# PaddleCV-SIG/MedicalSeg

Hardware: AMD Instinct MI355X
Metric: 3D-voxels/sec fwd+bwd, VNet 128^3 fp32 (higher is better)
Workload: dtype f32

## Files before the change

include/msegk.h:

```cpp
#ifndef MSEGK_H
#define MSEGK_H

#include <stddef.h>
#include <stdint.h>

#ifdef __cplusplus
extern "C" {
#endif

typedef struct msk_ctx msk_ctx;

typedef struct {
  void* p;
  int32_t n, d, h, w, c;
  int32_t ld;
} msk_tensor;

typedef struct {
  int32_t kd, kh, kw;
  int32_t sd, sh, sw;
  int32_t pd, ph, pw;
} msk_conv_desc;

int msk_version(void);
// ... 95 lines not shown
                               msk_tensor dy_scratch, msk_tensor dx, int dx_accumulate, float* dw, int dw_accumulate,
                               const void* xform , void* ybuf , const float* maxes ,
                               msk_tensor dx_lo, msk_tensor dx_hi, int* split_done);
int msk_conv3d_bwd_bnact_acc(msk_ctx* ctx, msk_conv_desc cd, msk_tensor x, const float* w, msk_tensor y, const float* scale,
                             const float* shift, const float* alpha, const float* mean, const float* invstd, const float* gamma,
                             msk_tensor dout, const float* sums_total, double M_total, msk_tensor dy_scratch, msk_tensor dx,
                             int dx_accumulate, float* dw, int dw_accumulate, const void* xform, void* ybuf, const float* maxes,
                             msk_tensor dx_old, msk_tensor dx_lo, msk_tensor dx_hi, int* split_done);
int msk_conv3d_bwd_bnact_join(msk_ctx* ctx, msk_conv_desc cd, msk_tensor x, const float* w, msk_tensor y, const float* scale,
                              const float* shift, const float* alpha , const float* mean, const float* invstd,
                              const float* gamma, msk_tensor dout, const float* sums_total, double M_total, msk_tensor dy,
                              float* dy_amax , float* dw, int dw_accumulate, const void* xform ,
                              const float* x_amax , msk_tensor jy, const float* jscale, const float* jshift,
                              const float* jalpha_inner, msk_tensor jres, const float* jalpha_outer, const float* jmean,
                              const float* jinvstd, msk_tensor da, int da_accumulate, msk_tensor dres ,
                              int dres_accumulate, float* dalpha_outer, float* unit_sums, float* maxes, int clear_maxes,
                              float* unit_dgamma , float* unit_dbeta , float* unit_dalpha );
int msk_convT3d_bwd_bnact(msk_ctx* ctx, msk_conv_desc cd, msk_tensor x, const float* w, msk_tensor y, const float* scale,
                          const float* shift, const float* alpha , const float* mean, const float* invstd,
                          msk_tensor dout, const float* sums_total, double M_total, msk_tensor dy_scratch, msk_tensor dx,
                          int dx_accumulate, float* dw, int dw_accumulate);
int msk_conv3d_bwd_inact(msk_ctx* ctx, msk_conv_desc cd, msk_tensor x, const float* w, msk_tensor y, const float* scale,
                         const float* shift, const float* alpha , const float* mean, const float* invstd, int coef_stride,
                         msk_tensor dout, const float* sums, int sums_stride, double M_sample, msk_tensor dx, int dx_accumulate,
                         float* dw, int dw_accumulate, const void* xform, void* ybuf, const float* maxes );
int msk_conv3d_bwd_bnact_c1(msk_ctx* ctx, msk_conv_desc cd, msk_tensor x, msk_tensor y, const float* scale, const float* shift,
                            const float* alpha , const float* mean, const float* invstd, msk_tensor res,
                            msk_tensor dout, const float* sums_total, double M_total, float* dw, int dw_accumulate);
int msk_conv3d_dgrad(msk_ctx* ctx, msk_conv_desc cd, msk_tensor dy, const float* w,
                     msk_tensor dx, int accumulate);
int msk_conv3d_wgrad(msk_ctx* ctx, msk_conv_desc cd, msk_tensor x, msk_tensor dy,
                     float* dw, float* db , int accumulate);
int msk_convT3d_fwd(msk_ctx* ctx, msk_conv_desc cd, msk_tensor x, const float* w,
                    const float* bias , msk_tensor y);
int msk_convT3d_fwd_ex(msk_ctx* ctx, msk_conv_desc cd, msk_tensor x, const float* w, const float* bias, msk_tensor y,
                       float* stats_local, const msk_bn_fin* fin );
int msk_convT3d_dgrad(msk_ctx* ctx, msk_conv_desc cd, msk_tensor dy, const float* w,
                      msk_tensor dx, int accumulate);
int msk_convT3d_wgrad(msk_ctx* ctx, msk_conv_desc cd, msk_tensor x, msk_tensor dy,
                      float* dw, float* db , int accumulate);

int msk_bn_stats(msk_ctx* ctx, msk_tensor x, float* stats_local);
int msk_bn_finalize(msk_ctx* ctx, const float* gathered, int world, double count_per_rank,
                    int C, const float* gamma, const float* beta, float eps, float momentum,
                    float* running_mean, float* running_var, float* save_mean,
                    float* save_invstd, float* scale, float* shift);
int msk_bn_eval_coeffs(msk_ctx* ctx, int C, const float* gamma, const float* beta,
                       const float* running_mean, const float* running_var, float eps,
                       float* save_mean, float* save_invstd, float* scale, float* shift);
int msk_affine_act_fwd(msk_ctx* ctx, msk_tensor x, const float* scale, const float* shift,
                       msk_tensor res, const float* alpha, msk_tensor out);
int msk_affine_act_fwd_amax2(msk_ctx* ctx, msk_tensor x, const float* scale, const float* shift, msk_tensor res,
                             const float* alpha, msk_tensor out, float* out_amax , msk_tensor out2);
int msk_affine_act_bwd_reduce(msk_ctx* ctx, msk_tensor x, const float* scale, const float* shift,
                              msk_tensor res, const float* alpha, const float* mean,
                              const float* invstd, msk_tensor dout, float* sums);
int msk_affine_act_bwd_reduce_ex(msk_ctx* ctx, msk_tensor x, const float* scale, const float* shift,
                                 msk_tensor res, const float* alpha, const float* mean,
                                 const float* invstd, msk_tensor dout, float* sums, float* maxes );
int msk_affine_act_bwd_apply(msk_ctx* ctx, msk_tensor x, const float* scale, const float* shift,
                             msk_tensor res, const float* alpha, const float* mean,
                             const float* invstd, const float* gamma, msk_tensor dout,
                             const float* sums_total, double M_total, int bn_mode,
                             msk_tensor dx, msk_tensor dres, int dres_acc);
int msk_affine_act_bwd_apply_amax(msk_ctx* ctx, msk_tensor x, const float* scale, const float* shift,
                                  msk_tensor res, const float* alpha, const float* mean,
                                  const float* invstd, const float* gamma, msk_tensor dout,
                                  const float* sums_total, double M_total, int bn_mode,
                                  msk_tensor dx, msk_tensor dres, int dres_acc, float* dx_amax );
int msk_affine_act_param_grads(msk_ctx* ctx, int C, const float* sums, float* dgamma,
                               float* dbeta, float* dalpha, int accumulate);

int msk_copy_scale(msk_ctx* ctx, msk_tensor src, const float* mask, msk_tensor dst, int accumulate);
int msk_dropout_mask(msk_ctx* ctx, uint64_t seed, uint64_t step, uint32_t site, int count,
                     float p, float* mask);
int msk_channel_sum(msk_ctx* ctx, msk_tensor x, float* out, int accumulate);
int msk_argmax_c(msk_ctx* ctx, msk_tensor x, int32_t* out);
int msk_softmax_c(msk_ctx* ctx, msk_tensor x, msk_tensor out);

int msk_flip_axes(msk_ctx* ctx, msk_tensor src, msk_tensor dst, int mask);
int msk_tta_accumulate(msk_ctx* ctx, msk_tensor logits, int mask, msk_tensor acc, int first);
int msk_tta_finish(msk_ctx* ctx, msk_tensor acc, int passes, msk_tensor probs, int32_t* pred);

int msk_sw_gather(msk_ctx* ctx, msk_tensor vol, msk_tensor patches, const int32_t* origins, float cval);
int msk_sw_accumulate(msk_ctx* ctx, msk_tensor logits, const int32_t* origins, const float* td, int nd, const float* th, int nh,
                      const float* tw, int nw, msk_tensor acc);
int msk_sw_gather_mirrored(msk_ctx* ctx, msk_tensor vol, msk_tensor patches, const int32_t* origins, float cval);
int msk_sw_accumulate_mirrored(msk_ctx* ctx, msk_tensor logits, const int32_t* origins, const float* td, int nd, const float* th,
                               int nh, const float* tw, int nw, float scale, msk_tensor acc);

int msk_patch_workspace(long voxels, int num_classes, size_t* bytes);
int msk_patch_select(msk_ctx* ctx, const int32_t* label, int d, int h, int w, int num_classes, const int32_t* classes,
                     int n_classes, int rd, int rh, int rw, const uint32_t* words, int n_patches, void* workspace,
                     int32_t* sel, int32_t* counts);
int msk_patch_crop(msk_ctx* ctx, const void* src, int d, int h, int w, const int32_t* sel, void* dst, int rd, int rh, int rw,
                   uint32_t pad_bits);

int msk_affine_patch(msk_ctx* ctx, const float* img, const int32_t* label, int d, int h, int w, const int32_t* sel,
                     const float* matrix, float* out_img, int32_t* out_label, int rd, int rh, int rw, float pad,
                     int32_t label_pad);
int msk_elastic_field(msk_ctx* ctx, uint64_t seed, int rd, int rh, int rw, const float* taps, int r, float alpha, int axes_mask,
                      float* field, float* scratch);
int msk_affine_patch_elastic(msk_ctx* ctx, const float* img, const int32_t* label, int d, int h, int w, const int32_t* sel,
                             const float* matrix, const float* field, float* out_img, int32_t* out_label, int rd, int rh, int rw,
                             float pad, int32_t label_pad);

#define MSK_INTENSITY_NOISE 0
#define MSK_INTENSITY_SCALE 1
#define MSK_INTENSITY_CONTRAST 2
#define MSK_INTENSITY_GAMMA 3
#define MSK_INTENSITY_RESTORE 4
int msk_intensity_stats_workspace(long n, size_t* bytes);
int msk_intensity_stats(msk_ctx* ctx, const float* x, long n, void* workspace, double* stats);
int msk_intensity_apply(msk_ctx* ctx, const float* x, float* y, long n, int mode, const float* params, const double* stats_a,
                        const double* stats_b, uint64_t seed);
int msk_gauss_blur3d(msk_ctx* ctx, const float* x, float* y, int d, int h, int w, const float* taps_d, int r_d,
                     const float* taps_h, int r_h, const float* taps_w, int r_w, float* tmp);

int msk_class_weights(msk_ctx* ctx, msk_tensor logits, float* weights);
int msk_loss_fwd(msk_ctx* ctx, msk_tensor logits, const int32_t* labels, const float* weights,
                 int ignore_index, float* out, double* stats);
int msk_loss_bwd(msk_ctx* ctx, msk_tensor logits, const int32_t* labels, const float* weights,
                 int ignore_index, const double* stats, float coef_ce, float coef_dice,
                 msk_tensor dlogits);

int msk_loss_fwd_ex(msk_ctx* ctx, msk_tensor logits, const int32_t* labels, const float* weights,
                    int ignore_index, int dice_softmax, const float* dice_weight, float* out, double* stats);
int msk_loss_bwd_ex(msk_ctx* ctx, msk_tensor logits, const int32_t* labels, const float* weights,
// ... 157 lines not shown
```

medicalseg_amd/_lib.py:

```python
from __future__ import annotations

import ctypes as C
import os

_HERE = os.path.dirname(os.path.abspath(__file__))
LIB_PATH = os.environ.get("MSEGK_LIB") or os.path.join(_HERE, "lib", "libmsegk.so")


class MskError(RuntimeError):
    pass


class MskTensor(C.Structure):
    _fields_ = [("p", C.c_void_p), ("n", C.c_int32), ("d", C.c_int32), ("h", C.c_int32),
                ("w", C.c_int32), ("c", C.c_int32), ("ld", C.c_int32)]


class MskConvDesc(C.Structure):
    _fields_ = [("kd", C.c_int32), ("kh", C.c_int32), ("kw", C.c_int32),
                ("sd", C.c_int32), ("sh", C.c_int32), ("sw", C.c_int32),
                ("pd", C.c_int32), ("ph", C.c_int32), ("pw", C.c_int32)]


class MskBnFin(C.Structure):
    _fields_ = [("gamma", C.c_void_p), ("beta", C.c_void_p), ("eps", C.c_float), ("momentum", C.c_float),
                ("count", C.c_double), ("running_mean", C.c_void_p), ("running_var", C.c_void_p),
                ("save_mean", C.c_void_p), ("save_invstd", C.c_void_p), ("scale", C.c_void_p), ("shift", C.c_void_p)]


NULL_TENSOR = MskTensor(None, 0, 0, 0, 0, 0, 0)

_vp, _i, _f, _d, _sz = C.c_void_p, C.c_int, C.c_float, C.c_double, C.c_size_t
_u64, _u32 = C.c_uint64, C.c_uint32
_T, _CD = MskTensor, MskConvDesc

SIGNATURES = {
    "msk_version": (_i, []),
    "msk_device_count": (_i, [C.POINTER(_i)]),
    "msk_ctx_create": (_i, [_i, C.POINTER(_vp)]),
    "msk_ctx_destroy": (_i, [_vp]),
    "msk_last_error": (C.c_char_p, [_vp]),
    "msk_sync": (_i, [_vp]),
    "msk_join_side": (_i, [_vp]),
    "msk_device_name": (_i, [_vp, C.c_char_p, _i]),
    "msk_device_pci_bus_id": (_i, [_vp, C.c_char_p, _i]),
    "msk_malloc": (_i, [_vp, _sz, C.POINTER(_vp)]),
    "msk_free": (_i, [_vp, _vp]),
    "msk_memset": (_i, [_vp, _vp, _i, _sz]),
    "msk_weights_changed": (_i, [_vp, _vp, _sz]),
    "msk_h2d": (_i, [_vp, _vp, _vp, _sz]),
    "msk_d2h": (_i, [_vp, _vp, _vp, _sz]),
    "msk_h2d_async": (_i, [_vp, _vp, _vp, _sz]),
    "msk_d2d": (_i, [_vp, _vp, _vp, _sz]),
    "msk_pinned_alloc": (_i, [_vp, _sz, C.POINTER(_vp)]),
    "msk_pinned_free": (_i, [_vp, _vp]),
    "msk_mem_info": (_i, [_vp, C.POINTER(_sz), C.POINTER(_sz)]),
    "msk_timer_start": (_i, [_vp]),
    "msk_timer_stop": (_i, [_vp, C.POINTER(_f)]),
    "msk_mark": (_i, [_vp, _i]),
    "msk_ctx_wait": (_i, [_vp, _vp]),
    "msk_mark_elapsed": (_i, [_vp, _i, _i, C.POINTER(_f)]),
    "msk_prof_enable": (_i, [_vp, _i]),
    "msk_prof_reset": (_i, [_vp]),
    "msk_prof_report": (_i, [_vp, C.c_char_p, _i, C.POINTER(_i)]),
    "msk_set_option": (_i, [_vp, C.c_char_p, _i]),
    "msk_get_option": (_i, [_vp, C.c_char_p, C.POINTER(_i)]),
    "msk_ncdhw_to_ndhwc": (_i, [_vp, _vp, _T]),
    "msk_ndhwc_to_ncdhw": (_i, [_vp, _T, _vp]),
    "msk_conv3d_fwd": (_i, [_vp, _CD, _T, _vp, _vp, _T]),
    "msk_conv_fold_bn": (_i, [_vp, _vp, _vp, _vp, _vp, _i, C.c_long, _vp, _vp]),
    "msk_conv3d_fwd_act": (_i, [_vp, _CD, _T, _vp, _vp, _vp, _T]),
    "msk_conv3d_xform_bytes": (_sz, [_vp, _CD, _T, _i]),
    "msk_conv3d_fwd_ex": (_i, [_vp, _CD, _T, _vp, _vp, _T, _vp, _vp]),
    "msk_conv3d_wgrad_ex": (_i, [_vp, _CD, _T, _T, _vp, _vp, _i, _vp]),
    "msk_amax_new": (_vp, [_vp, _i]),
    "msk_conv3d_fwd_ex3": (_i, [_vp, _CD, _T, _vp, _vp, _T, _vp, _vp, _vp, _vp]),
    "msk_conv3d_fwd_in": (_i, [_vp, _CD, _T, _vp, _vp, _T, _vp, _vp, _vp, _vp, _i]),
    "msk_bn_stats_fin": (_i, [_vp, _T, _vp, _vp]),
    "msk_affine_act_bwd_reduce_pg": (_i, [_vp, _T, _vp, _vp, _T, _vp, _vp, _vp, _T, _vp, _vp, _i, _vp, _vp, _vp]),
    "msk_add_act_join_bwd_pg": (_i, [_vp, _T, _vp, _vp, _vp, _T, _vp, _vp, _vp, _T, _T, _T, _i, _vp, _vp, _vp, _i, _vp, _vp, _vp]),
    "msk_conv3d_fwd_ex2": (_i, [_vp, _CD, _T, _vp, _vp, _T, _vp, _vp, _vp]),
    "msk_affine_act_fwd_amax": (_i, [_vp, _T, _vp, _vp, _T, _vp, _T, _vp]),
    "msk_affine_act_fwd_amax2": (_i, [_vp, _T, _vp, _vp, _T, _vp, _T, _vp, _T]),
    "msk_affine_act_join_fwd_amax": (_i, [_vp, _T, _vp, _vp, _vp, _T, _vp, _T, _vp]),
    "msk_copy_scale_amax": (_i, [_vp, _T, _vp, _T, _i, _vp]),
    "msk_conv3d_bwd_bnact_bytes": (_sz, [_vp, _CD, _T, _T]),
    "msk_conv3d_bwd_bnact": (_i, [_vp, _CD, _T, _vp, _T, _vp, _vp, _vp, _vp, _vp, _vp, _T, _vp, _d, _T, _T, _i, _vp, _i, _vp, _vp, _vp]),
    "msk_convT3d_bwd_bnact": (_i, [_vp, _CD, _T, _vp, _T, _vp, _vp, _vp, _vp, _vp, _T, _vp, _d, _T, _T, _i, _vp, _i]),
    "msk_conv3d_bwd_bnact_split": (_i, [_vp, _CD, _T, _vp, _T, _vp, _vp, _vp, _vp, _vp, _vp, _T, _vp, _d, _T, _T, _i, _vp, _i, _vp, _vp, _vp, _T, _T, C.POINTER(_i)]),
    "msk_conv3d_bwd_bnact_acc": (_i, [_vp, _CD, _T, _vp, _T, _vp, _vp, _vp, _vp, _vp, _vp, _T, _vp, _d, _T, _T, _i, _vp, _i, _vp, _vp, _vp, _T, _T, _T, C.POINTER(_i)]),
    "msk_conv3d_bwd_inact": (_i, [_vp, _CD, _T, _vp, _T, _vp, _vp, _vp, _vp, _vp, _i, _T, _vp, _i, _d, _T, _i, _vp, _i, _vp, _vp, _vp]),
    "msk_conv3d_bwd_bnact_join": (_i, [_vp, _CD, _T, _vp, _T, _vp, _vp, _vp, _vp, _vp, _vp, _T, _vp, _d, _T, _vp, _vp, _i, _vp, _vp,
                                       _T, _vp, _vp, _vp, _T, _vp, _vp, _vp, _T, _i, _T, _i, _vp, _vp, _vp, _i, _vp, _vp, _vp]),
    "msk_conv3d_bwd_bnact_c1": (_i, [_vp, _CD, _T, _T, _vp, _vp, _vp, _vp, _vp, _T, _T, _vp, _d, _vp, _i]),
    "msk_conv3d_dgrad": (_i, [_vp, _CD, _T, _vp, _T, _i]),
    "msk_conv3d_dgrad_ex": (_i, [_vp, _CD, _T, _vp, _T, _i, _vp]),
    "msk_conv3d_wgrad_ex2": (_i, [_vp, _CD, _T, _T, _vp, _vp, _i, _vp, _vp]),
    "msk_conv3d_wgrad_ex3": (_i, [_vp, _CD, _T, _T, _vp, _vp, _i, _vp, _vp, _vp]),
    "msk_conv3d_wgrad": (_i, [_vp, _CD, _T, _T, _vp, _vp, _i]),
    "msk_convT3d_fwd": (_i, [_vp, _CD, _T, _vp, _vp, _T]),
    "msk_convT3d_fwd_ex": (_i, [_vp, _CD, _T, _vp, _vp, _T, _vp, _vp]),
    "msk_convT3d_dgrad": (_i, [_vp, _CD, _T, _vp, _T, _i]),
    "msk_convT3d_wgrad": (_i, [_vp, _CD, _T, _T, _vp, _vp, _i]),
    "msk_bn_stats": (_i, [_vp, _T, _vp]),
    "msk_bn_finalize": (_i, [_vp, _vp, _i, _d, _i, _vp, _vp, _f, _f, _vp, _vp, _vp, _vp, _vp, _vp]),
    "msk_bn_eval_coeffs": (_i, [_vp, _i, _vp, _vp, _vp, _vp, _f, _vp, _vp, _vp, _vp]),
    "msk_affine_act_fwd": (_i, [_vp, _T, _vp, _vp, _T, _vp, _T]),
    "msk_affine_act_bwd_reduce": (_i, [_vp, _T, _vp, _vp, _T, _vp, _vp, _vp, _T, _vp]),
    "msk_affine_act_bwd_reduce_ex": (_i, [_vp, _T, _vp, _vp, _T, _vp, _vp, _vp, _T, _vp, _vp]),
    "msk_affine_act_bwd_apply": (_i, [_vp, _T, _vp, _vp, _T, _vp, _vp, _vp, _vp, _T, _vp, _d, _i, _T, _T, _i]),
    "msk_affine_act_bwd_apply_amax": (_i, [_vp, _T, _vp, _vp, _T, _vp, _vp, _vp, _vp, _T, _vp, _d, _i, _T, _T, _i, _vp]),
    "msk_affine_act_param_grads": (_i, [_vp, _i, _vp, _vp, _vp, _vp, _i]),
    "msk_add_act_bwd": (_i, [_vp, _T, _T, _vp, _T, _T, _T, _i, _vp]),
    "msk_affine_act_join_fwd": (_i, [_vp, _T, _vp, _vp, _vp, _T, _vp, _T]),
    "msk_add_act_join_bwd": (_i, [_vp, _T, _vp, _vp, _vp, _T, _vp, _T, _T, _T, _i, _vp]),
    "msk_add_act_join_bwd_ex": (_i, [_vp, _T, _vp, _vp, _vp, _T, _vp, _vp, _vp, _T, _T, _T, _i, _vp, _vp, _vp]),
    "msk_bn_bias_grad": (_i, [_vp, _i, _vp, _vp, _vp, _i]),
    "msk_copy_scale": (_i, [_vp, _T, _vp, _T, _i]),
    "msk_dropout_mask": (_i, [_vp, _u64, _u64, _u32, _i, _f, _vp]),
    "msk_channel_sum": (_i, [_vp, _T, _vp, _i]),
    "msk_argmax_c": (_i, [_vp, _T, _vp]),
    "msk_softmax_c": (_i, [_vp, _T, _T]),
    "msk_flip_axes": (_i, [_vp, _T, _T, _i]),
    "msk_tta_accumulate": (_i, [_vp, _T, _i, _T, _i]),
    "msk_tta_finish": (_i, [_vp, _T, _i, _T, _vp]),
    "msk_sw_gather": (_i, [_vp, _T, _T, _vp, _f]),
    "msk_sw_accumulate": (_i, [_vp, _T, _vp, _vp, _i, _vp, _i, _vp, _i, _T]),
    "msk_sw_gather_mirrored": (_i, [_vp, _T, _T, _vp, _f]),
    "msk_sw_accumulate_mirrored": (_i, [_vp, _T, _vp, _vp, _i, _vp, _i, _vp, _i, _f, _T]),
    "msk_patch_workspace": (_i, [C.c_long, _i, C.POINTER(_sz)]),
    "msk_patch_select": (_i, [_vp, _vp, _i, _i, _i, _i, _vp, _i, _i, _i, _i, _vp, _i, _vp, _vp, _vp]),
    "msk_patch_crop": (_i, [_vp, _vp, _i, _i, _i, _vp, _vp, _i, _i, _i, _u32]),
    "msk_affine_patch": (_i, [_vp, _vp, _vp, _i, _i, _i, _vp, _vp, _vp, _vp, _i, _i, _i, _f, C.c_int32]),
    "msk_elastic_field": (_i, [_vp, _u64, _i, _i, _i, _vp, _i, _f, _i, _vp, _vp]),
    "msk_affine_patch_elastic": (_i, [_vp, _vp, _vp, _i, _i, _i, _vp, _vp, _vp, _vp, _vp, _i, _i, _i, _f, C.c_int32]),
    "msk_intensity_stats_workspace": (_i, [C.c_long, C.POINTER(_sz)]),
    "msk_intensity_stats": (_i, [_vp, _vp, C.c_long, _vp, _vp]),
    "msk_intensity_apply": (_i, [_vp, _vp, _vp, C.c_long, _i, _vp, _vp, _vp, _u64]),
    "msk_gauss_blur3d": (_i, [_vp, _vp, _vp, _i, _i, _i, _vp, _i, _vp, _i, _vp, _i, _vp]),
    "msk_class_weights": (_i, [_vp, _T, _vp]),
    "msk_loss_fwd": (_i, [_vp, _T, _vp, _vp, _i, _vp, _vp]),
    "msk_loss_bwd": (_i, [_vp, _T, _vp, _vp, _i, _vp, _f, _f, _T]),
    "msk_elu_fwd": (_i, [_vp, _T, _f, _T]),
    "msk_elu_bwd": (_i, [_vp, _T, _T, _f, _T, _i]),
    "msk_loss_fwd_ex": (_i, [_vp, _T, _vp, _vp, _i, _i, _vp, _vp, _vp]),
    "msk_loss_bwd_ex": (_i, [_vp, _T, _vp, _vp, _i, _i, _vp, _vp, _f, _f, _T]),
    "msk_bce_fwd": (_i, [_vp, _T, _vp, _i, _i, _i, _f, _vp, _vp]),
    "msk_bce_bwd": (_i, [_vp, _T, _vp, _i, _vp, _f, _i, _T]),
    "msk_region_loss_fwd": (_i, [_vp, _T, _vp, _i, _i, _i, _i, _i, _i, _f, _f, _f, _i, _f, _vp, _vp, _vp]),
    "msk_region_loss_bwd": (_i, [_vp, _T, _vp, _i, _i, _i, _i, _i, _i, _f, _f, _f, _i, _f, _vp, _vp, _f, _f, _i, _T]),
    "msk_mlabel_loss_fwd": (_i, [_vp, _T, _vp, _i, _vp, _i, _i, _i, _f, _vp, _vp]),
    "msk_mlabel_loss_bwd": (_i, [_vp, _T, _vp, _i, _vp, _i, _i, _i, _f, _vp, _f, _f, _i, _T]),
    "msk_regions_to_label": (_i, [_vp, _T, _vp, _vp]),
    "msk_topk_workspace": (_i, [C.c_long, C.POINTER(_sz)]),
    "msk_topk_select": (_i, [_vp, _vp, C.c_long, C.c_long, _vp, _vp]),
    "msk_topk_ce_fwd": (_i, [_vp, _T, _vp, _i, _vp, _f, _vp, _vp, _vp]),
    "msk_topk_ce_bwd": (_i, [_vp, _T, _vp, _i, _vp, _vp, _vp, _f, _i, _T]),
    "msk_fg_stats_workspace": (_i, [C.c_long, C.POINTER(_sz)]),
    "msk_fg_stats": (_i, [_vp, _vp, _vp, C.c_long, _i, _d, _d, _vp, _vp]),
    "msk_clip_zscore": (_i, [_vp, _vp, _vp, C.c_long, _i, _vp, _vp, _i, _f, _vp]),
    "msk_nonzero_bbox": (_i, [_vp, _vp, _i, _i, _i, _i, _vp]),
    "msk_sdf_workspace": (_i, [_i, _i, _i, C.POINTER(_sz)]),
    "msk_label_sdf": (_i, [_vp, _vp, _i, _i, _i, _i, _u64, _vp, _vp, _sz, _vp]),
    "msk_boundary_loss_fwd": (_i, [_vp, _T, _vp, _i, _u64, _vp, _vp, _vp]),
    "msk_boundary_loss_bwd": (_i, [_vp, _T, _vp, _i, _u64, _vp, _vp, _f, _i, _T]),
    "msk_sgd_momentum": (_i, [_vp, _vp, _vp, _vp, _sz, _f, _f, _f, _f]),
    "msk_sgd_momentum_eager": (_i, [_vp, _vp, _vp, _vp, _sz, _f, _f, _f, _f]),
    "msk_sgd_momentum_finish": (_i, [_vp]),
    "msk_adam": (_i, [_vp, _vp, _vp, _vp, _vp, _sz, _f, _f, _f, _f, _d, _d, _f, _f]),
    "msk_grad_clip_workspace": (_i, [_sz, C.POINTER(_sz)]),
    "msk_grad_clip_coef": (_i, [_vp, _vp, _sz, _f, _f, _vp, _vp]),
    "msk_sgd_momentum_clip": (_i, [_vp, _vp, _vp, _vp, _sz, _f, _f, _f, _f, _i, _vp, _f, _f]),
# ... 76 lines not shown
```

medicalseg_amd/csrc/msk_common.h:

```cpp
#pragma once
#include <hip/hip_runtime.h>
#include <hip/hip_ext.h>

#include <cstdint>
#include <cstdio>
#include <cstring>
#include <map>
#include <set>
#include <string>
#include <utility>
#include <vector>

#include "msegk.h"

struct msk_prof_entry {
  double total_ms = 0.0;
  long calls = 0;
};

struct msk_pending_event {
  hipEvent_t a, b;
  const char* tag;
};

// ... 54 lines not shown
  int wbf_pack_lds = 1;
  int wbf_bpf = 1;
  int wbf_fused_sh = 1;
  int wbf_gemm_form = -1;
  int wbf_ks_blocks = 2;
  int noop_after_merge = 0;
  int wgrad_c1_wpc = 2;
  int eager_tail_main = 1;
  int prof_paused = 0;
  int prof_attach = 1;
  int small_pack_cache = 1;
  int wbf_prepack = 1;
  int ks_legacy = 0;
  int wgrad_fork = 1;
  int wbf_fused_bl = 2;
  int wbf_fuse = 1;
  int conv_split = 2;
  int bwd_fuse = -1;
  int foldn_wgs = 0;
  int wgrad_wino_rounds = 0;
  int wgrad_rounds = 8;
  int poison = -1;
  hipStream_t side = nullptr;
  void* ws_side = nullptr;
  size_t ws_side_bytes = 0;
  void* ws3_side = nullptr;
  size_t ws3_side_bytes = 0;
  hipEvent_t ev_fork = nullptr, ev_join = nullptr;
  hipEvent_t ev_late = nullptr;
  bool late_valid = false;
  const float* late_ptr = nullptr;
  size_t late_count = 0;
  float* late_alpha = nullptr;
  struct { float* param = nullptr; const float* grad = nullptr; float* velocity = nullptr; size_t count = 0;
           float lr = 0, momentum = 0, weight_decay = 0, grad_scale = 0; } late_piece;
  int late_split = 1;
  bool wgrad_async = false;
  bool side_dirty = false;
  hipEvent_t fork_event = nullptr;
  int fork_attach = 1;
  bool fork_recorded = false;
  void* stage[2] = {nullptr, nullptr};
  size_t stage_bytes[2] = {0, 0};
  hipEvent_t stage_ev[2] = {nullptr, nullptr};
  int stage_next = 0;
  void* comm = nullptr;
  void* comm_grad = nullptr;
  hipStream_t comm_stream = nullptr;
  hipEvent_t ev_comm_main = nullptr, ev_comm_side = nullptr, ev_comm_done = nullptr, ev_comm_back = nullptr;
  int c1_h2 = 1;
  int dst_split = 1;
  int wgrad_reduce_rows = 1;
  int ks_stats = 1;
  int ks_lds = 1;
  int ks_nr_max = 4;
  int wgrad_lds_pad = 0;
  int kst_pair = 1;
  int tile_staging = 7;
  int wgrad_renorm = 1;
  int dy_bound_shift = 0;
  int dp_mode = 0;
  bool comm_pending = false;
  bool host_transport = false;
  std::vector<int> host_fds;
  int rank = 0, world = 1;
  int tk_join = 1;
  int topk_agg_hist = 0;
  int affine_map = 1;
  int num_cu = 256;
};

extern thread_local std::string g_msk_global_err;

int msk_fail(msk_ctx* ctx, const char* file, int line, const char* what, const char* detail);
void* msk_workspace(msk_ctx* ctx, size_t bytes);
void* msk_workspace2(msk_ctx* ctx, size_t bytes);
void* msk_workspace3(msk_ctx* ctx, size_t bytes);
hipEvent_t msk_prof_event(msk_ctx* ctx);
void msk_prof_begin(msk_ctx* ctx, const char* tag);
void msk_prof_end(msk_ctx* ctx);
const char* msk_intern_tag(msk_ctx* ctx, const std::string& s);
int msk_join_side_impl(msk_ctx* ctx);
void msk_set_dense12(int v);
void msk_set_reduce_vpl(int v);
void msk_set_reduce_vpl_site(int v);
void msk_set_ew_caps(int ew, int red);
int msk_get_ew_option(const char* key, int* value);
void msk_weights_changed_impl(msk_ctx* ctx, const void* p, size_t bytes);
void msk_weights_freed_impl(msk_ctx* ctx, const void* p, size_t bytes);
int msk_prepack_impl(msk_ctx* ctx);
int msk_prepack_range_impl(msk_ctx* ctx, const void* p, size_t bytes);
int msk_dp_wait_impl(msk_ctx* ctx);
int msk_edt_field(msk_ctx* ctx, const int32_t* vol, int d, int h, int w, int cls, int surface_only, int complement,
                  const double* spacing, double* dist2);
int msk_join_sums_merge(msk_ctx* ctx, const float* partial, int nb, int C, float* unit_sums, float* u_dbeta, float* u_dgamma,
                        float* u_dalpha, float* dalpha);

struct msk_side_scope {
  msk_ctx* ctx;
  bool active;
  explicit msk_side_scope(msk_ctx* c, bool want = true) : ctx(c), active(want && c->wgrad_async && c->side != nullptr) {
    const bool forked = ctx->fork_recorded;
    hipEvent_t fev = forked && ctx->fork_event ? ctx->fork_event : ctx->ev_fork;
    ctx->fork_recorded = false;
    ctx->fork_event = nullptr;
    if (!active) return;
// ... 84 lines not shown
```

medicalseg_amd/csrc/msk_conv_ksfwd.hip:

```cpp
#include "msk_conv.h"
#ifdef KS_PROBE_NOMFMA
#define __builtin_amdgcn_mfma_f32_32x32x2f32(a_, b_, c_, x_, y_, z_) ks_probe_keep((a_), (b_), (c_))
#define __builtin_amdgcn_mfma_f32_16x16x4f32(a_, b_, c_, x_, y_, z_) ks_probe_keep((a_), (b_), (c_))
template <typename T> __device__ __forceinline__ T ks_probe_keep(float a, float b, T c) { asm volatile("" ::"v"(a), "v"(b)); c[0] += a * 1e-30f + b * 1e-30f; return c; }
#endif

typedef float f32x16 __attribute__((ext_vector_type(16)));

namespace {

constexpr unsigned kOOBk = 0xFFFFFFF0u;

struct KsBnBwd {
  const float* y;
  const float* dout;
  int yld, dld;
  unsigned y_bytes, d_bytes;
  const float *scale, *shift, *alpha, *mean, *invstd, *sums;
  float invM;
};

template <int NR, int KB, bool FUSE = false>
__global__ void __launch_bounds__(256, FUSE ? 2 : (NR == 1 ? 4 : (NR == 2 ? 4 : 2)))
gconv_ks_fwd_k(GConv g, const float4* __restrict__ wm, int KC, int npad, unsigned src_bytes, KsBnBwd bn) {
  const int tid = threadIdx.x;
  const int wave = tid >> 6, lane = tid & 63, li = lane & 31, lh = lane >> 5;
  const long M = (long)g.N * g.DD * g.DH * g.DW;
  const long m = ((long)blockIdx.x * 4 + wave) * 32 + li;
  if (((long)blockIdx.x * 4 + wave) * 32 >= M) return;
  const bool mok = m < M;
  unsigned ow, oh, od, n;
  {
    const unsigned r = (unsigned)(mok ? m : 0);
    const unsigned t1 = r / (unsigned)g.DW, t2 = t1 / (unsigned)g.DH;
    ow = r - t1 * (unsigned)g.DW;
    oh = t1 - t2 * (unsigned)g.DH;
    n = t2 / (unsigned)g.DD;
    od = t2 - n * (unsigned)g.DD;
  }
  const unsigned vox0 = ((n * g.SD + od * g.sd) * g.SH + oh * g.sh) * g.SW + ow * g.sw;
  const unsigned xbase = mok ? (vox0 * (unsigned)g.sld + lh * 4u) * 4u : kOOBk;
  const __amdgpu_buffer_rsrc_t rs = __builtin_amdgcn_make_buffer_rsrc((void*)(FUSE ? bn.y : g.src), 0, FUSE ? bn.y_bytes : src_bytes, 0x00020000);
  const unsigned ybase = mok ? (vox0 * (unsigned)bn.yld + lh * 4u) * 4u : kOOBk;
  const unsigned dbase = mok ? (vox0 * (unsigned)bn.dld + lh * 4u) * 4u : kOOBk;
  const __amdgpu_buffer_rsrc_t rd = __builtin_amdgcn_make_buffer_rsrc((void*)(FUSE ? bn.dout : g.src), 0, FUSE ? bn.d_bytes : src_bytes, 0x00020000);
  float c_sc[2][4], c_sf[2][4], c_al[2][4], c_mu[2][4], c_is[2][4], c_s1[2][4], c_s2[2][4];
  if constexpr (FUSE) {
#pragma unroll
    for (int k = 0; k < 2; ++k)
#pragma unroll
      for (int j = 0; j < 4; ++j) {
        const int c = k * 8 + lh * 4 + j;
        const bool ok = c < g.CK;
        c_sc[k][j] = ok ? bn.scale[c] : 0.f;
        c_sf[k][j] = ok ? bn.shift[c] : 0.f;
        c_al[k][j] = (ok && bn.alpha) ? bn.alpha[c] : 1.f;
        c_mu[k][j] = ok ? bn.mean[c] : 0.f;
        c_is[k][j] = ok ? bn.invstd[c] : 0.f;
        c_s1[k][j] = ok ? bn.sums[c] * bn.invM : 0.f;
        c_s2[k][j] = ok ? bn.sums[g.CK + c] * bn.invM : 0.f;
      }
  }
  const int nt0 = blockIdx.y * NR;
  const int T = g.kd * g.kh * g.kw * KC;
  const float4* wl = wm + (long)lh * npad + nt0 * 32 + li;

  f32x16 acc[NR];
#pragma unroll
  for (int r = 0; r < NR; ++r)
#pragma unroll
    for (int j = 0; j < 16; ++j) acc[r][j] = 0.f;

  float4 xa[KB], xb[KB], wa[KB][NR], wb[KB][NR];
  int lt = 0, lkc = 0, lta = 0, ltb = 0, ltc = 0;
  auto load = [&](float4 (&xv)[KB], float4 (&wv)[KB][NR]) {
#pragma unroll
    for (int u = 0; u < KB; ++u) {
      const bool tin = lt < T;
      const unsigned soff = (unsigned)((((lta * g.SH + ltb) * g.SW + ltc) * g.sld + lkc * 8) * 4);
      const bool live = tin && lkc * 8 + lh * 4 < g.CK;
      if constexpr (FUSE) {
        const unsigned tvox = (unsigned)((lta * g.SH + ltb) * g.SW + ltc);
// ... 3 lines not shown
        const float on = live ? 1.f : 0.f;
        const int k = lkc & 1;
        float o[4];
#pragma unroll
        for (int j = 0; j < 4; ++j) {
          const float sc = k ? c_sc[1][j] : c_sc[0][j], sf = k ? c_sf[1][j] : c_sf[0][j], al = k ? c_al[1][j] : c_al[0][j];
          const float mu = k ? c_mu[1][j] : c_mu[0][j], is = k ? c_is[1][j] : c_is[0][j];
          const float s1 = k ? c_s1[1][j] : c_s1[0][j], s2 = k ? c_s2[1][j] : c_s2[0][j];
          float d = dv[j];
          if (bn.alpha) {
            const float uu = fmaf(yv[j], sc, sf);
            if (!(uu > 0.f)) d *= al;
          }
          const float xh = (yv[j] - mu) * is;
          o[j] = on * (sc * (d - s1 - xh * s2));
        }
        xv[u] = make_float4(o[0], o[1], o[2], o[3]);
      } else {
        xv[u] = __builtin_bit_cast(float4, __builtin_amdgcn_raw_buffer_load_b128(rs, (int)(live ? xbase : kOOBk), (int)(tin ? soff : 0u), 0));
      }
#pragma unroll
      for (int r = 0; r < NR; ++r) wv[u][r] = tin ? wl[(long)lt * 2 * npad + r * 32] : make_float4(0.f, 0.f, 0.f, 0.f);
      ++lt;
      if (++lkc == KC) {
        lkc = 0;
        if (++ltc == g.kw) {
          ltc = 0;
          if (++ltb == g.kh) {
            ltb = 0;
            ++lta;
          }
        }
      }
    }
  };
  auto compute = [&](const float4 (&xv)[KB], const float4 (&wv)[KB][NR]) {
#pragma unroll
    for (int u = 0; u < KB; ++u)
#pragma unroll
      for (int r = 0; r < NR; ++r) {
        acc[r] = __builtin_amdgcn_mfma_f32_32x32x2f32(wv[u][r].x, xv[u].x, acc[r], 0, 0, 0);
        acc[r] = __builtin_amdgcn_mfma_f32_32x32x2f32(wv[u][r].y, xv[u].y, acc[r], 0, 0, 0);
        acc[r] = __builtin_amdgcn_mfma_f32_32x32x2f32(wv[u][r].z, xv[u].z, acc[r], 0, 0, 0);
        acc[r] = __builtin_amdgcn_mfma_f32_32x32x2f32(wv[u][r].w, xv[u].w, acc[r], 0, 0, 0);
      }
  };
  load(xa, wa);
  for (int t0 = 0; t0 < T; t0 += 2 * KB) {
    load(xb, wb);
    compute(xa, wa);
    load(xa, wa);
    if (t0 + KB < T) compute(xb, wb);
  }
  if (!mok) return;

  float* orow = g.dst + m * g.dld;
#pragma unroll
  for (int r = 0; r < NR; ++r) {
    float4 old[4];
    bool ok[4];
#pragma unroll
    for (int q = 0; q < 4; ++q) {
      const int cn = (nt0 + r) * 32 + 8 * q + 4 * lh;
      ok[q] = cn < g.CN;
      old[q] = (g.accumulate && ok[q]) ? *reinterpret_cast<const float4*>(orow + cn) : make_float4(0.f, 0.f, 0.f, 0.f);
    }
#pragma unroll
    for (int q = 0; q < 4; ++q) {
      if (ok[q]) {
        const int cn = (nt0 + r) * 32 + 8 * q + 4 * lh;
        const float4 bv = g.bias ? make_float4(g.bias[cn], g.bias[cn + 1], g.bias[cn + 2], g.bias[cn + 3]) : make_float4(0.f, 0.f, 0.f, 0.f);
        float4 v;
        v.x = acc[r][4 * q + 0] + bv.x + old[q].x;
        v.y = acc[r][4 * q + 1] + bv.y + old[q].y;
        v.z = acc[r][4 * q + 2] + bv.z + old[q].z;
        v.w = acc[r][4 * q + 3] + bv.w + old[q].w;
        *reinterpret_cast<float4*>(orow + cn) = v;
      }
    }
  }
}

#ifndef KS_DBG
#define KS_DBG 0
#endif
template <int NR, int CK, bool FUSE>
__global__ void __launch_bounds__(256, 3)
gconv_ks_lds_k(GConv g, const float4* __restrict__ wm, int npad, KsBnBwd bn, int runs) {
  constexpr int KC = CK / 8, QV = CK / 4;
  constexpr int PP = 2 * CK * 4 + 16;
  constexpr int ROWB = 32 * PP;
  constexpr int NL = 64 * QV / 64;
  __shared__ __attribute__((aligned(16))) char lds[4 * 2 * ROWB];
  const int tid = threadIdx.x;
  const int wave = __builtin_amdgcn_readfirstlane(tid >> 6), lane = tid & 63, li = lane & 31, lh = lane >> 5;
  const int rid = blockIdx.x * 4 + wave;
  if (rid >= runs) return;
  char* reg = lds + wave * 2 * ROWB;
  const int rpr = g.DW / 32;
  int t = rid / rpr;
  const int ow0 = (rid - t * rpr) * 32;
  const int oh = t % g.DH;
  t /= g.DH;
  const int od = t % g.DD, n = t / g.DD;
  const long m = (((long)n * g.DD + od) * g.DH + oh) * g.DW + ow0 + li;
  const int nt0 = blockIdx.y * NR;
  const float4* wl = wm + (long)lh * npad + nt0 * 32 + li;

  const int jq = lane % QV;
  float c_sc[4], c_sf[4], c_al[4], c_mu[4], c_is[4], c_s1[4], c_s2[4];
  if constexpr (FUSE) {
#pragma unroll
    for (int j = 0; j < 4; ++j) {
      const int c = jq * 4 + j;
      c_sc[j] = bn.scale[c];
      c_sf[j] = bn.shift[c];
      c_al[j] = bn.alpha ? bn.alpha[c] : 1.f;
      c_mu[j] = bn.mean[c];
      c_is[j] = bn.invstd[c];
      c_s1[j] = bn.sums[c] * bn.invM;
      c_s2[j] = bn.sums[CK + c] * bn.invM;
    }
  }
  const int sld = FUSE ? bn.yld : g.sld;
  const float* sp = FUSE ? bn.y : g.src;
  float4 xa[2][NL], xd[2][NL];
  auto issue = [&](int a) {
#pragma unroll
    for (int b = 0; b < 2; ++b) {
      const long v0 = (((long)n * g.SD + 2 * od + a) * g.SH + 2 * oh + b) * g.SW + 2 * ow0;
#pragma unroll
      for (int i = 0; i < NL; ++i) {
        const int q = lane + 64 * i, v = q / QV;
        xa[b][i] = (KS_DBG & 8) ? make_float4((float)v, 1.f, 2.f, 3.f) : *reinterpret_cast<const float4*>(sp + (v0 + v) * sld + jq * 4);
        if constexpr (FUSE) xd[b][i] = *reinterpret_cast<const float4*>(bn.dout + (v0 + v) * bn.dld + jq * 4);
      }
    }
  };
  auto commit = [&]() {
#pragma unroll
    for (int b = 0; b < 2; ++b)
#pragma unroll
      for (int i = 0; i < NL; ++i) {
        const int q = lane + 64 * i, v = q / QV;
        float4 o = xa[b][i];
        if constexpr (FUSE) {
          const float yv[4] = {o.x, o.y, o.z, o.w}, dv[4] = {xd[b][i].x, xd[b][i].y, xd[b][i].z, xd[b][i].w};
          float r[4];
#pragma unroll
          for (int j = 0; j < 4; ++j) {
// ... 13 lines not shown

  f32x16 acc[NR];
#pragma unroll
  for (int r = 0; r < NR; ++r)
#pragma unroll
    for (int j = 0; j < 16; ++j) acc[r][j] = 0.f;

  issue(0);
#pragma unroll
  for (int a = 0; a < 2; ++a) {
    commit();
    if (a == 0) issue(1);
#pragma unroll
    for (int b = 0; b < 2; ++b)
#pragma unroll
      for (int c = 0; c < 2; ++c)
#pragma unroll
        for (int kc = 0; kc < KC; ++kc) {
          const int tap = (a * 2 + b) * 2 + c;
          const float4 xq = *reinterpret_cast<const float4*>(reg + b * ROWB + li * PP + c * (CK * 4) + kc * 32 + lh * 16);
#pragma unroll
          for (int r = 0; r < NR; ++r) {
            const float4 wq = (KS_DBG & 2) ? make_float4((float)(tap + kc + r), 0.5f, 0.25f, 2.f) : wl[(long)(tap * KC + kc) * 2 * npad + r * 32];
            if (KS_DBG & 1) {
              acc[r][(tap + kc) & 15] += wq.x * xq.x + wq.y * xq.y + wq.z * xq.z + wq.w * xq.w;
              continue;
            }
            acc[r] = __builtin_amdgcn_mfma_f32_32x32x2f32(wq.x, xq.x, acc[r], 0, 0, 0);
            acc[r] = __builtin_amdgcn_mfma_f32_32x32x2f32(wq.y, xq.y, acc[r], 0, 0, 0);
            acc[r] = __builtin_amdgcn_mfma_f32_32x32x2f32(wq.z, xq.z, acc[r], 0, 0, 0);
            acc[r] = __builtin_amdgcn_mfma_f32_32x32x2f32(wq.w, xq.w, acc[r], 0, 0, 0);
          }
        }
  }

  float* orow = g.dst + m * g.dld;
#pragma unroll
  for (int r = 0; r < NR; ++r) {
    float4 old[4];
#pragma unroll
    for (int q = 0; q < 4; ++q) {
      const int cn = (nt0 + r) * 32 + 8 * q + 4 * lh;
      old[q] = g.accumulate ? *reinterpret_cast<const float4*>(orow + cn) : make_float4(0.f, 0.f, 0.f, 0.f);
    }
#pragma unroll
    for (int q = 0; q < 4; ++q) {
      const int cn = (nt0 + r) * 32 + 8 * q + 4 * lh;
      const float4 bv = g.bias ? make_float4(g.bias[cn], g.bias[cn + 1], g.bias[cn + 2], g.bias[cn + 3]) : make_float4(0.f, 0.f, 0.f, 0.f);
      float4 v;
      v.x = acc[r][4 * q + 0] + bv.x + old[q].x;
      v.y = acc[r][4 * q + 1] + bv.y + old[q].y;
      v.z = acc[r][4 * q + 2] + bv.z + old[q].z;
      v.w = acc[r][4 * q + 3] + bv.w + old[q].w;
      if (!(KS_DBG & 4) || v.x == 12345.678f) *reinterpret_cast<float4*>(orow + cn) = v;
    }
  }
}

template <int NR, int KB, bool PAIR = false>
__global__ void __launch_bounds__(256, NR == 1 ? 4 : (NR == 2 ? 4 : 2))
gconv_kst_k(GConv g, const float4* __restrict__ wm, int KC, int npad, unsigned src_bytes, int waves_per_class) {
  const int tid = threadIdx.x;
  const int wave = tid >> 6, lane = tid & 63, li = lane & 31, lh = lane >> 5;
  const long gw = (long)blockIdx.x * 4 + wave;
  const int cls = (int)(gw / waves_per_class);
  if (cls >= (PAIR ? g.sd : g.sd * g.sh)) return;
  const int ra = PAIR ? cls : cls / g.sh, rb = PAIR ? 0 : cls - ra * g.sh;
  const long per_class = (long)g.N * g.SD * g.SH * g.DW;
  const long q = (gw - (long)cls * waves_per_class) * 32 + li;
  const bool mok = q < per_class;
  unsigned W, h, d, n;
  {
    const unsigned r = (unsigned)(mok ? q : 0);
    const unsigned t1 = r / (unsigned)g.DW, t2 = t1 / (unsigned)g.SH;
    W = r - t1 * (unsigned)g.DW;
    h = t1 - t2 * (unsigned)g.SH;
    n = t2 / (unsigned)g.SD;
    d = t2 - n * (unsigned)g.SD;
  }
  const unsigned xrow = (((n * g.SD + d) * g.SH + h) * g.SW) * (unsigned)g.sld + lh * 4u;
  const __amdgpu_buffer_rsrc_t rs = __builtin_amdgcn_make_buffer_rsrc((void*)g.src, 0, src_bytes, 0x00020000);
  const int nt0 = blockIdx.y * NR;
  const int T = g.kw * KC;
  const float4* wl = PAIR ? wm + ((long)(ra * g.kh + (li >> 4)) * g.kw * KC) * 2 * npad + (long)lh * npad + (li & 15)
                          : wm + ((long)(ra * g.kh + rb) * g.kw * KC) * 2 * npad + (long)lh * npad + nt0 * 32 + li;

  f32x16 acc[NR];
#pragma unroll
  for (int r = 0; r < NR; ++r)
#pragma unroll
    for (int j = 0; j < 16; ++j) acc[r][j] = 0.f;

  float4 xa[KB], xb[KB], wa[KB][NR], wb[KB][NR];
  int lt = 0, lkc = 0, ltc = 0;
  auto load = [&](float4 (&xv)[KB], float4 (&wv)[KB][NR]) {
#pragma unroll
    for (int u = 0; u < KB; ++u) {
      const bool tin = lt < T;
      const int sw_ = (int)W - ltc;
      const bool live = tin && mok && sw_ >= 0 && sw_ < g.SW && lkc * 8 + lh * 4 < g.CK;
      const unsigned voff = live ? (xrow + (unsigned)sw_ * (unsigned)g.sld) * 4u : kOOBk;
      xv[u] = __builtin_bit_cast(float4, __builtin_amdgcn_raw_buffer_load_b128(rs, (int)voff, (int)(tin ? lkc * 32 : 0), 0));
#pragma unroll
      for (int r = 0; r < NR; ++r) wv[u][r] = tin ? wl[(long)lt * 2 * npad + r * 32] : make_float4(0.f, 0.f, 0.f, 0.f);
      ++lt;
      if (++lkc == KC) {
        lkc = 0;
        ++ltc;
      }
// ... 81 lines not shown
  }
  msk_launch_scope ls(ctx, tag);
  dim3 grid((unsigned)blocks, ntn / NR);
  const float4* w4 = reinterpret_cast<const float4*>(wm);
  if (pair) {
    hipLaunchKernelGGL((gconv_kst_k<1, 4, true>), grid, dim3(256), 0, ctx->stream, g, w4, KC, npad, (unsigned)sbytes, (int)wpc);
    MSK_LAUNCH_CHECK(ctx);
    return 1;
  }
  switch (NR) {
    case 4: hipLaunchKernelGGL((gconv_kst_k<4, 2>), grid, dim3(256), 0, ctx->stream, g, w4, KC, npad, (unsigned)sbytes, (int)wpc); break;
    case 2: hipLaunchKernelGGL((gconv_kst_k<2, 2>), grid, dim3(256), 0, ctx->stream, g, w4, KC, npad, (unsigned)sbytes, (int)wpc); break;
    default: hipLaunchKernelGGL((gconv_kst_k<1, 4>), grid, dim3(256), 0, ctx->stream, g, w4, KC, npad, (unsigned)sbytes, (int)wpc); break;
  }
  MSK_LAUNCH_CHECK(ctx);
  return 1;
}

static int gconv_ks_fwd_impl(msk_ctx* ctx, const GConv& g, const float* w_canon, int A, int B, int swap, const KsBnBwd* bnp, bool dry = false);
int msk_gconv_ks_fwd(msk_ctx* ctx, const GConv& g, const float* w_canon, int A, int B, int swap) {
  return gconv_ks_fwd_impl(ctx, g, w_canon, A, B, swap, nullptr);
}
int msk_gconv_ks_fwd_bnbwd(msk_ctx* ctx, const GConv& g0, const float* w_canon, int A, int B, int swap, const float* y, int yld,
                           const float* dout, int dld, const float* scale, const float* shift, const float* alpha, const float* mean,
                           const float* invstd, const float* sums, double M_total, bool dry) {
  if (g0.CK > 16 || yld % 4 || dld % 4 || ((uintptr_t)y) % 16 || ((uintptr_t)dout) % 16) return 0;
  const size_t vox = (size_t)g0.N * g0.SD * g0.SH * g0.SW;
  if (vox * yld * sizeof(float) >= 0xFFFFFFF0ull || vox * dld * sizeof(float) >= 0xFFFFFFF0ull) return 0;
  KsBnBwd bn{};
  bn.y = y; bn.dout = dout; bn.yld = yld; bn.dld = dld;
  bn.y_bytes = (unsigned)(vox * yld * sizeof(float)); bn.d_bytes = (unsigned)(vox * dld * sizeof(float));
  bn.scale = scale; bn.shift = shift; bn.alpha = alpha; bn.mean = mean; bn.invstd = invstd; bn.sums = sums;
  bn.invM = (float)(1.0 / M_total);
  GConv g = g0;
  g.src = y; g.sld = yld;
  return gconv_ks_fwd_impl(ctx, g, w_canon, A, B, swap, &bn, dry);
}
static int gconv_ks_fwd_impl(msk_ctx* ctx, const GConv& g, const float* w_canon, int A, int B, int swap, const KsBnBwd* bnp, bool dry) {
  if (g.transposed) return 0;
  if (!(g.pd == 0 && g.ph == 0 && g.pw == 0)) return 0;
  if ((g.DD - 1) * g.sd + g.kd > g.SD || (g.DH - 1) * g.sh + g.kh > g.SH || (g.DW - 1) * g.sw + g.kw > g.SW) return 0;
  const int taps = g.kd * g.kh * g.kw;
  if (taps < 2 || (g.kd == 5 && g.kh == 5 && g.kw == 5)) return 0;
  if (g.CK % 4 || g.CN % 4 || g.sld % 4 || g.dld % 4 || ((uintptr_t)g.src) % 16 || ((uintptr_t)g.dst) % 16) return 0;
  const size_t sbytes = (size_t)g.N * g.SD * g.SH * g.SW * g.sld * sizeof(float);
  const long M = (long)g.N * g.DD * g.DH * g.DW;
  if (sbytes >= 0xFFFFFFF0ull || M >= (1L << 31)) return 0;
  if (dry) return 1;
  const int KC = (g.CK + 7) / 8;
  const int npad = ((g.CN + 31) / 32) * 32;
  const float* wm = msk_pack_weights_get(ctx, w_canon, A, B, taps, swap, 0, g.kd, g.kh, g.kw, 1, g.CK, g.CN, KC, npad);
  if (!wm) return -1;
  const int ntn = npad / 32;
  if (ctx->ks_lds && g.kd == 2 && g.kh == 2 && g.kw == 2 && g.sd == 2 && g.sh == 2 && g.sw == 2 && g.SD == 2 * g.DD && g.SH == 2 * g.DH &&
      g.SW == 2 * g.DW && g.DW % 32 == 0 && (g.CK == 8 || g.CK == 16) && g.CN % 32 == 0 && (!g.bias || ((uintptr_t)g.bias) % 16 == 0)) {
    const int runs = (int)(M / 32);
    const int NRl = ntn % 2 == 0 ? 2 : 1;
    const char* tag = bnp ? "gconv_ks_lds_bnbwd" : "gconv_ks_lds";
    if (ctx->prof && ctx->prof_shapes) {
      char buf[160];
      snprintf(buf, sizeof(buf), "%s[ck=%d,cn=%d,dst=%dx%dx%dx%d,sld=%d,dld=%d,acc=%d,nr=%d]", tag, g.CK, g.CN, g.N, g.DD, g.DH, g.DW, g.sld, g.dld,
               g.accumulate, NRl);
      tag = msk_intern_tag(ctx, buf);
    }
    msk_launch_scope ls(ctx, tag);
    const dim3 grid((unsigned)((runs + 3) / 4), ntn / NRl);
    const float4* w4 = reinterpret_cast<const float4*>(wm);
    const KsBnBwd bnv = bnp ? *bnp : KsBnBwd{};
#define KS_LDS(NR_, CK_) \
    do { \
      if (bnp) hipLaunchKernelGGL((gconv_ks_lds_k<NR_, CK_, true>), grid, dim3(256), 0, ctx->stream, g, w4, npad, bnv, runs); \
      else hipLaunchKernelGGL((gconv_ks_lds_k<NR_, CK_, false>), grid, dim3(256), 0, ctx->stream, g, w4, npad, bnv, runs); \
    } while (0)
    if (g.CK == 16) { if (NRl == 2) KS_LDS(2, 16); else KS_LDS(1, 16); }
    else { if (NRl == 2) KS_LDS(2, 8); else KS_LDS(1, 8); }
#undef KS_LDS
    MSK_LAUNCH_CHECK(ctx);
    return 1;
  }
  const long mtiles = (M + 127) / 128;
  int NR = ntn % 4 == 0 ? 4 : (ntn % 2 == 0 ? 2 : 1);
  while (NR > ctx->ks_nr_max) NR >>= 1;
  while (NR > 1 && mtiles * (ntn / NR) < 2L * ctx->num_cu) NR >>= 1;
  if (bnp && NR > 2) NR = 2;
  const char* tag = bnp ? "gconv_ks_fwd_bnbwd" : "gconv_ks_fwd";
  if (ctx->prof && ctx->prof_shapes) {
    char buf[160];
    snprintf(buf, sizeof(buf), "%s[ck=%d,cn=%d,k=%dx%dx%d,dst=%dx%dx%dx%d,sld=%d,dld=%d,acc=%d,nr=%d]", tag, g.CK, g.CN, g.kd, g.kh, g.kw, g.N, g.DD, g.DH,
             g.DW, g.sld, g.dld, g.accumulate, NR);
    tag = msk_intern_tag(ctx, buf);
  }
  msk_launch_scope ls(ctx, tag);
  dim3 grid((unsigned)mtiles, ntn / NR);
  const float4* w4 = reinterpret_cast<const float4*>(wm);
  switch (NR) {
    case 4:
      hipLaunchKernelGGL((gconv_ks_fwd_k<4, 2>), grid, dim3(256), 0, ctx->stream, g, w4, KC, npad, (unsigned)sbytes, KsBnBwd{});
      break;
    case 2:
      if (bnp) hipLaunchKernelGGL((gconv_ks_fwd_k<2, 2, true>), grid, dim3(256), 0, ctx->stream, g, w4, KC, npad, (unsigned)sbytes, *bnp);
      else hipLaunchKernelGGL((gconv_ks_fwd_k<2, 2>), grid, dim3(256), 0, ctx->stream, g, w4, KC, npad, (unsigned)sbytes, KsBnBwd{});
      break;
    default:
      if (bnp) hipLaunchKernelGGL((gconv_ks_fwd_k<1, 2, true>), grid, dim3(256), 0, ctx->stream, g, w4, KC, npad, (unsigned)sbytes, *bnp);
      else hipLaunchKernelGGL((gconv_ks_fwd_k<1, 4>), grid, dim3(256), 0, ctx->stream, g, w4, KC, npad, (unsigned)sbytes, KsBnBwd{});
      break;
  }
  MSK_LAUNCH_CHECK(ctx);
  return 1;
}
```

medicalseg_amd/csrc/msk_ctx.hip:

```cpp
#include <cstdlib>

#include "msk_common.h"

thread_local std::string g_msk_global_err;

int msk_fail(msk_ctx* ctx, const char* file, int line, const char* what, const char* detail) {
  char buf[1024];
  const char* base = strrchr(file, '/');
  snprintf(buf, sizeof(buf), "%s:%d: %s: %s", base ? base + 1 : file, line, what, detail ? detail : "");
  if (ctx) ctx->err = buf;
  g_msk_global_err = buf;
  return -1;
}

static void* grow(msk_ctx* ctx, void** p, size_t* cur, size_t bytes) {
  if (bytes <= *cur) return *p;
  if (*p) {
    hipStreamSynchronize(ctx->stream);
    hipFree(*p);
    *p = nullptr;
    *cur = 0;
  }
  size_t want = bytes + (bytes >> 2);
  if (hipMalloc(p, want) != hipSuccess) {
// ... 335 lines not shown
  return 0;
}
int msk_ctx_wait(msk_ctx* ctx, msk_ctx* other) {
  MSK_REQUIRE(ctx, other != nullptr && other->device == ctx->device, "msk_ctx_wait: two contexts on the same device");
  if (other == ctx) return 0;
  MSK_CHECK_HIP(ctx, hipSetDevice(ctx->device));
  if (!ctx->ev_xctx) MSK_CHECK_HIP(ctx, hipEventCreateWithFlags(&ctx->ev_xctx, hipEventDisableTiming));
  MSK_CHECK_HIP(ctx, hipEventRecord(ctx->ev_xctx, other->stream));
  MSK_CHECK_HIP(ctx, hipStreamWaitEvent(ctx->stream, ctx->ev_xctx, 0));
  return 0;
}
int msk_mark_elapsed(msk_ctx* ctx, int a, int b, float* ms) {
  MSK_REQUIRE(ctx, a >= 0 && b >= 0 && a < (int)ctx->marks.size() && b < (int)ctx->marks.size() && ctx->marks[a] && ctx->marks[b],
              "mark not recorded");
  MSK_CHECK_HIP(ctx, hipEventSynchronize(ctx->marks[b]));
  MSK_CHECK_HIP(ctx, hipEventElapsedTime(ms, ctx->marks[a], ctx->marks[b]));
  return 0;
}

int msk_prof_enable(msk_ctx* ctx, int on) {
  if (!on) drain_prof(ctx);
  ctx->prof = on != 0;
  return 0;
}
int msk_prof_reset(msk_ctx* ctx) {
  drain_prof(ctx);
  ctx->prof_map.clear();
  return 0;
}
int msk_prof_report(msk_ctx* ctx, char* buf, int buflen, int* len) {
  drain_prof(ctx);
  std::string s;
  char line[256];
  for (auto& kv : ctx->prof_map) {
    snprintf(line, sizeof(line), "%s\t%ld\t%.6f\n", kv.first.c_str(), kv.second.calls, kv.second.total_ms);
    s += line;
  }
  if (len) *len = (int)s.size() + 1;
  if (buf && buflen > 0) {
    strncpy(buf, s.c_str(), buflen - 1);
    buf[buflen - 1] = 0;
  }
  return 0;
}

int msk_get_option(msk_ctx* ctx, const char* key, int* value) {
  MSK_REQUIRE(ctx, key != nullptr && value != nullptr, "msk_get_option: null argument");
  if (strcmp(key, "dp_mode") == 0) *value = ctx->dp_mode;
  else if (strcmp(key, "conv_split") == 0) *value = ctx->conv_split;
  else if (strcmp(key, "wgrad_async") == 0) *value = ctx->wgrad_async ? 1 : 0;
  else if (strcmp(key, "world") == 0) *value = ctx->world;
  else if (strcmp(key, "rank") == 0) *value = ctx->rank;
  else if (strcmp(key, "num_cu") == 0) *value = ctx->num_cu;
  else if (strcmp(key, "scalar_ring_served") == 0) *value = (int)(ctx->scalar_served & 0x3FFFFFFF);
  else if (strcmp(key, "scalar_ring_served_side") == 0) *value = (int)(ctx->scalar_served_side & 0x3FFFFFFF);
  else if (msk_get_ew_option(key, value)) {}
  else return msk_fail(ctx, __FILE__, __LINE__, "msk_get_option", "unknown key");
  return 0;
}
int msk_set_option(msk_ctx* ctx, const char* key, int value) {
  if (strcmp(key, "conv_impl") == 0) {
    ctx->conv_impl = value;
    return 0;
  }
  if (strcmp(key, "halo_tile") == 0) {
    ctx->halo_tile = value;
    return 0;
  }
  if (strcmp(key, "prof_only_halo") == 0) {
    snprintf(ctx->prof_prefix, sizeof(ctx->prof_prefix), "%s", value ? (ctx->wbf ? "wbf_gemm_" : "conv_halo_") : "");
    return 0;
  }
  if (strcmp(key, "wgrad_async_max_m") == 0) {
    ctx->wgrad_async_max_m = value;
    return 0;
  }
  if (strcmp(key, "wino_bf3") == 0) {
    ctx->wbf = value != 0;
    return 0;
  }
  if (strcmp(key, "conv_fp16") == 0) {
    ctx->conv_fp16 = value != 0;
    return 0;
  }
  if (strcmp(key, "wbf_tin_map") == 0) {
    ctx->wbf_tin_map = value;
    return 0;
  }
  if (strcmp(key, "wbf_mr4") == 0) {
    ctx->wbf_mr4 = value;
    return 0;
  }
  if (strcmp(key, "wbf_variant") == 0) {
    ctx->wbf_variant = value;
    return 0;
  }
  if (strcmp(key, "direct_conv") == 0) {
    ctx->no_winograd = value != 0;
    return 0;
  }
  if (strcmp(key, "wbf_tin_groups") == 0) {
    ctx->wbf_tin_groups = value;
    return 0;
  }
  if (strcmp(key, "wbf_pad_min_voxels") == 0) {
    ctx->wbf_pad_min_voxels = value > 0 ? value : 0;
// ... 25 lines not shown
  }
  if (strcmp(key, "wgrad_c1_wpc") == 0) {
    ctx->wgrad_c1_wpc = value < 1 ? 1 : value;
    return 0;
  }
  if (strcmp(key, "eager_tail_main") == 0) {
    ctx->eager_tail_main = value;
    return 0;
  }
  if (strcmp(key, "fork_attach") == 0) {
    ctx->fork_attach = value;
    return 0;
  }
  if (strcmp(key, "prof_paused") == 0) {
    ctx->prof_paused = value;
    return 0;
  }
  if (strcmp(key, "prof_attach") == 0) {
    ctx->prof_attach = value;
    return 0;
  }
  if (strcmp(key, "noop_after_merge") == 0) {
    ctx->noop_after_merge = value;
    return 0;
  }
  if (strcmp(key, "small_pack_cache") == 0) {
    ctx->small_pack_cache = value;
    return 0;
  }
  if (strcmp(key, "wbf_prepack") == 0) {
    ctx->wbf_prepack = value;
    return 0;
  }
  if (strcmp(key, "dp_mode") == 0) {
    if (value < 0 || value > 3 || (value == 2 && ctx->comm != nullptr && ctx->comm_grad == nullptr))
      return msk_fail(ctx, __FILE__, __LINE__, "msk_set_option", "dp_mode: 0, 1, 2 or 3 (2 only before msk_dp_init)");
    ctx->dp_mode = value;
    return 0;
  }
  if (strcmp(key, "ew_cap") == 0) {
    msk_set_ew_caps(value, 0);
    return 0;
  }
  if (strcmp(key, "dst_split") == 0) {
    ctx->dst_split = value;
    return 0;
  }
  if (strcmp(key, "wgrad_reduce_rows") == 0) {
    ctx->wgrad_reduce_rows = value;
    return 0;
  }
  if (strcmp(key, "ks_stats") == 0) {
    ctx->ks_stats = value;
    return 0;
  }
  if (strcmp(key, "ks_lds") == 0) {
    ctx->ks_lds = value;
    return 0;
  }
  if (strcmp(key, "dense12") == 0) {
    msk_set_dense12(value);
    return 0;
  }
  if (strcmp(key, "reduce_vpl") == 0) {
    msk_set_reduce_vpl(value);
    return 0;
  }
  if (strcmp(key, "reduce_vpl_site") == 0) {
    msk_set_reduce_vpl_site(value);
    return 0;
  }
  if (strcmp(key, "reduce_cap") == 0) {
    msk_set_ew_caps(0, value);
    return 0;
  }
  if (strcmp(key, "dy_bound_shift") == 0) {
    ctx->dy_bound_shift = value;
    return 0;
  }
  if (strcmp(key, "late_split") == 0) {
    ctx->late_split = value != 0;
    return 0;
  }
  if (strcmp(key, "c1_h2") == 0) {
    ctx->c1_h2 = value < 0 ? 0 : (value > 2 ? 2 : value);
    return 0;
  }
  if (strcmp(key, "ks_nr_max") == 0) {
    ctx->ks_nr_max = value >= 4 ? 4 : (value >= 2 ? 2 : 1);
    return 0;
  }
  if (strcmp(key, "wgrad_lds_pad") == 0) {
    ctx->wgrad_lds_pad = value > 0 ? value : 0;
    return 0;
  }
  if (strcmp(key, "kst_pair") == 0) {
    ctx->kst_pair = value != 0;
    return 0;
  }
  if (strcmp(key, "tile_staging") == 0) {
    ctx->tile_staging = value;
    return 0;
  }
  if (strcmp(key, "wgrad_renorm") == 0) {
    ctx->wgrad_renorm = value != 0;
    return 0;
// ... 80 lines not shown
```

medicalseg_amd/csrc/msk_elementwise.hip:

```cpp
#include "msk_common.h"
#include "msk_wbf.h"

namespace {

constexpr int kThreads = 256;

inline int pow2ceil(int v) {
  int p = 1;
  while (p < v) p <<= 1;
  return p;
}

struct ChanGeom {
  int CB, VPB, cblocks;
};
inline ChanGeom chan_geom(int C) {
  ChanGeom g;
  g.CB = pow2ceil(C) < kThreads ? pow2ceil(C) : kThreads;
  g.VPB = kThreads / g.CB;
  g.cblocks = (C + g.CB - 1) / g.CB;
  return g;
}

#ifndef EW_LB
// ... 266 lines not shown
  } else {
    v = i / cv;
    cg = (int)(i - v * cv);
  }
}


template <int V>
__global__ void __launch_bounds__(kThreads)
affine_act_fwd_k(const float* __restrict__ x, int ldx, const float* __restrict__ scale,
                 const float* __restrict__ shift, const float* __restrict__ res, int ldr, int cres,
                 const float* __restrict__ alpha, float* __restrict__ out, int ldo, long voxels, int C,
                 const float* __restrict__ alpha_in, unsigned* __restrict__ out_amax) {
  const int cv = C / V;
  const int cshift = (cv & (cv - 1)) == 0 ? __ffs(cv) - 1 : -1;
  const long total = voxels * cv;
  float mx = 0.f;
  for (long i = (long)blockIdx.x * blockDim.x + threadIdx.x; i < total; i += (long)gridDim.x * blockDim.x) {
    long v;
    int cg;
    split_vc(i, cv, cshift, v, cg);
    const int c = cg * V;
    float xv[V], o[V];
    ldv<V>(x + v * ldx + c, xv);
#pragma unroll
    for (int j = 0; j < V; ++j) {
      float u = xv[j];
      if (scale) u = fmaf(u, scale[c + j], shift[c + j]);
      if (alpha_in && !(u > 0.f)) u *= alpha_in[c + j];
      o[j] = u;
    }
    if (res) {
      if (cres == C) {
        float rv[V];
        ldv<V>(res + v * ldr + c, rv);
#pragma unroll
        for (int j = 0; j < V; ++j) o[j] += rv[j];
      } else {
#pragma unroll
        for (int j = 0; j < V; ++j) o[j] += res[v * ldr + (c + j) % cres];
      }
    }
    if (alpha) {
#pragma unroll
      for (int j = 0; j < V; ++j) o[j] = o[j] > 0.f ? o[j] : alpha[c + j] * o[j];
    }
#pragma unroll
    for (int j = 0; j < V; ++j) mx = fmaxf(mx, fabsf(o[j]));
    stv<V>(out + v * ldo + c, o);
  }
  if (out_amax) block_atomic_max(out_amax, mx);
}

__global__ void EW_BOUNDS
affine_act_fwd_cs_k(const float* __restrict__ x, int ldx, const float* __restrict__ scale,
                    const float* __restrict__ shift, const float* __restrict__ res, int ldr, int cres,
                    const float* __restrict__ alpha, float* __restrict__ out, int ldo, long voxels, int C, int cshift,
                    const float* __restrict__ alpha_in, unsigned* __restrict__ out_amax, float* __restrict__ out2, int ldo2) {
  float mx = 0.f;
  const long g = (long)blockIdx.x * kThreads + threadIdx.x;
  const int c = (int)(g & ((C >> 2) - 1)) * 4;
  const long vstride = ((long)gridDim.x * kThreads) >> cshift;
  float sc[4], sf[4], al[4], ai[4];
#pragma unroll
  for (int j = 0; j < 4; ++j) {
    sc[j] = scale ? scale[c + j] : 1.f;
    sf[j] = scale ? shift[c + j] : 0.f;
    al[j] = alpha ? alpha[c + j] : 1.f;
    ai[j] = alpha_in ? alpha_in[c + j] : 1.f;
  }
  auto load_res = [&](long v) {
    if (!res) return make_float4(0.f, 0.f, 0.f, 0.f);
    if (cres == C) return *reinterpret_cast<const float4*>(res + v * ldr + c);
    const float* r = res + v * ldr;
    if (cres == 1) {
      const float r0 = r[0];
      return make_float4(r0, r0, r0, r0);
    }
    return make_float4(r[c % cres], r[(c + 1) % cres], r[(c + 2) % cres], r[(c + 3) % cres]);
  };
  auto body = [&](long v, const float4 xq, const float4 rq) {
    const float xv[4] = {xq.x, xq.y, xq.z, xq.w}, rv[4] = {rq.x, rq.y, rq.z, rq.w};
    float o[4];
#pragma unroll
    for (int j = 0; j < 4; ++j) {
      float t = fmaf(xv[j], sc[j], sf[j]);
      if (alpha_in && !(t > 0.f)) t *= ai[j];
      const float u = t + rv[j];
      o[j] = (alpha && !(u > 0.f)) ? al[j] * u : u;
    }
    mx = fmaxf(fmaxf(mx, fmaxf(fabsf(o[0]), fabsf(o[1]))), fmaxf(fabsf(o[2]), fabsf(o[3])));
    *reinterpret_cast<float4*>(out + v * ldo + c) = make_float4(o[0], o[1], o[2], o[3]);
    if (out2) *reinterpret_cast<float4*>(out2 + v * ldo2 + c) = make_float4(o[0], o[1], o[2], o[3]);
  };
  long v = g >> cshift;
  for (; v + vstride < voxels; v += 2 * vstride) {
    const float4 xa = *reinterpret_cast<const float4*>(x + v * ldx + c);
    const float4 xb = *reinterpret_cast<const float4*>(x + (v + vstride) * ldx + c);
    const float4 ra = load_res(v), rb = load_res(v + vstride);
    body(v, xa, ra);
    body(v + vstride, xb, rb);
  }
  if (v < voxels) body(v, *reinterpret_cast<const float4*>(x + v * ldx + c), load_res(v));
  if (out_amax) block_atomic_max(out_amax, mx);
}

__global__ void __launch_bounds__(kThreads)
affine_act_bwd_reduce_k(const float* __restrict__ x, int ldx, const float* __restrict__ scale,
                        const float* __restrict__ shift, const float* __restrict__ res, int ldr,
                        int cres, const float* __restrict__ alpha, const float* __restrict__ mean,
                        const float* __restrict__ invstd, const float* __restrict__ dout, int ldd,
                        long voxels, int C, int CB, int VPB, float* __restrict__ partial ) {
  __shared__ float sh[3][kThreads];
  const int t = threadIdx.x;
  const int cl = t % CB, vl = t / CB;
  const int c = blockIdx.y * CB + cl;
  const int nb = gridDim.x;
  const long per = (voxels + nb - 1) / nb;
  const long v0 = (long)blockIdx.x * per;
  long v1 = v0 + per;
  if (v1 > voxels) v1 = voxels;
  float s_du = 0.f, s_dux = 0.f, s_da = 0.f;
  if (c < C) {
    const float sc = scale ? scale[c] : 1.f, sf = scale ? shift[c] : 0.f;
    const float al = alpha ? alpha[c] : 1.f;
    const float mu = mean ? mean[c] : 0.f, is = mean ? invstd[c] : 0.f;
    const int cr = res ? (cres == C ? c : c % cres) : 0;
    for (long v = v0 + vl; v < v1; v += VPB) {
      float xv = x[v * ldx + c];
      float u = fmaf(xv, sc, sf);
      if (res) u += res[v * ldr + cr];
      float d = dout[v * ldd + c];
      float du = d;
      if (alpha && !(u > 0.f)) {
        du = al * d;
        s_da = fmaf(d, u, s_da);
      }
      s_du += du;
      s_dux = fmaf(du, (xv - mu) * is, s_dux);
    }
  }
  sh[0][t] = s_du;
  sh[1][t] = s_dux;
  sh[2][t] = s_da;
  __syncthreads();
  for (int s = VPB >> 1; s > 0; s >>= 1) {
    if (vl < s) {
      sh[0][t] += sh[0][t + s * CB];
      sh[1][t] += sh[1][t + s * CB];
      sh[2][t] += sh[2][t + s * CB];
    }
    __syncthreads();
  }
  if (vl == 0) {
    float* p = partial + ((long)blockIdx.y * nb + blockIdx.x) * 3 * CB;
    p[cl] = sh[0][t];
    p[CB + cl] = sh[1][t];
// ... 339 lines not shown
    const int c = cg * V;
    float s[V];
    ldv<V>(src + v * lds_ + c, s);
    if (mask) {
      const long n = v / vox_per_n;
#pragma unroll
      for (int j = 0; j < V; ++j) s[j] *= mask[n * C + c + j];
    }
    if (acc) {
      float a[V];
      ldv<V>(dst + v * ldd + c, a);
#pragma unroll
      for (int j = 0; j < V; ++j) s[j] += a[j];
    }
#pragma unroll
    for (int j = 0; j < V; ++j) mx = fmaxf(mx, fabsf(s[j]));
    stv<V>(dst + v * ldd + c, s);
  }
  if (dst_amax) block_atomic_max(dst_amax, mx);
}

__global__ void __launch_bounds__(kThreads)
channel_sum_partial_k(const float* __restrict__ x, int ldx, long voxels, int C, int CB, int VPB,
                      float* __restrict__ partial ) {
  __shared__ float sh[kThreads];
  const int t = threadIdx.x;
  const int cl = t % CB, vl = t / CB;
  const int c = blockIdx.y * CB + cl;
  const int nb = gridDim.x;
  const long per = (voxels + nb - 1) / nb;
  const long v0 = (long)blockIdx.x * per;
  long v1 = v0 + per;
  if (v1 > voxels) v1 = voxels;
  float s = 0.f;
  if (c < C)
    for (long v = v0 + vl; v < v1; v += VPB) s += x[v * ldx + c];
  sh[t] = s;
  __syncthreads();
  for (int k = VPB >> 1; k > 0; k >>= 1) {
    if (vl < k) sh[t] += sh[t + k * CB];
    __syncthreads();
  }
  if (vl == 0) partial[((long)blockIdx.y * nb + blockIdx.x) * CB + cl] = sh[t];
}

__global__ void dropout_mask_k(uint64_t seed, uint64_t step, uint32_t site, int count, float p, float* mask) {
  int i = blockIdx.x * blockDim.x + threadIdx.x;
  if (i >= count) return;
  uint64_t h = splitmix64(seed ^ splitmix64(step * 0x100000001B3ull + site));
  h = splitmix64(h + (uint64_t)i);
  float u = (float)(h >> 40) * (1.0f / 16777216.0f);
  mask[i] = u >= p ? 1.0f / (1.0f - p) : 0.f;
}

__global__ void argmax_k(const float* __restrict__ x, int ld, long voxels, int C, int32_t* __restrict__ out) {
  for (long v = (long)blockIdx.x * blockDim.x + threadIdx.x; v < voxels; v += (long)gridDim.x * blockDim.x) {
    const float* p = x + v * ld;
    float best = p[0];
    int bi = 0;
    for (int c = 1; c < C; ++c) {
      float q = p[c];
      if (q > best) {
        best = q;
        bi = c;
      }
    }
    out[v] = bi;
  }
}

__global__ void softmax_c_k(const float* __restrict__ x, int ld, long voxels, int C, float* __restrict__ out, int old) {
  for (long v = (long)blockIdx.x * blockDim.x + threadIdx.x; v < voxels; v += (long)gridDim.x * blockDim.x) {
    const float* p = x + v * ld;
    float m = p[0];
    for (int c = 1; c < C; ++c) m = fmaxf(m, p[c]);
    float s = 0.f;
    for (int c = 0; c < C; ++c) s += expf(p[c] - m);
    const float inv = 1.f / s;
    float* o = out + v * old;
    for (int c = 0; c < C; ++c) o[c] = expf(p[c] - m) * inv;
  }
}

__global__ void __launch_bounds__(256)
ncdhw_to_ndhwc_k(const float* __restrict__ src, float* __restrict__ dst, int ld, long V, int C) {
  __shared__ float tile[32][33];
  const long n = blockIdx.z;
  const long v0 = (long)blockIdx.x * 32;
  const int c0 = blockIdx.y * 32;
  const int tx = threadIdx.x % 32, ty = threadIdx.x / 32;
  for (int r = ty; r < 32; r += 8) {
    int c = c0 + r;
    long v = v0 + tx;
    tile[r][tx] = (c < C && v < V) ? src[(n * C + c) * V + v] : 0.f;
  }
  __syncthreads();
  for (int r = ty; r < 32; r += 8) {
    long v = v0 + r;
    int c = c0 + tx;
    if (c < C && v < V) dst[(n * V + v) * ld + c] = tile[tx][r];
  }
}
__global__ void __launch_bounds__(256)
ndhwc_to_ncdhw_k(const float* __restrict__ src, int ld, float* __restrict__ dst, long V, int C) {
  __shared__ float tile[32][33];
  const long n = blockIdx.z;
// ... 368 lines not shown

int msk_bn_stats(msk_ctx* ctx, msk_tensor x, float* stats_local) { return msk_bn_stats_fin(ctx, x, stats_local, nullptr); }

int msk_bn_stats_fin(msk_ctx* ctx, msk_tensor x, float* stats_local, const msk_bn_fin* fin) {
  const long voxels = msk_voxels(x);
  MSK_REQUIRE(ctx, voxels > 0 && x.c > 0, "empty tensor");
  const ReducePlan p = reduce_plan(PassTensors{x}, voxels, ctx->num_cu, 0);
  float* partial = (float*)msk_workspace(ctx, p.bytes(3));
  if (!partial) return -1;
  {
    msk_launch_scope ls(ctx, "bn_stats_partial");
    if (p.form == RedForm::V4) {
      hipLaunchKernelGGL(bn_stats_partial_v4, dim3(p.nb), dim3(kThreads), 0, ctx->stream, (const float*)x.p, voxels, x.c,
                         x.ld, p.lanes, p.rows, partial);
    } else if (p.form == RedForm::D12) {
      const long groups = voxels * x.c / 12;
      d12_ladder(x.c, [&](auto c) {
        hipLaunchKernelGGL(bn_stats_partial_d12_k<decltype(c)::value>, dim3(p.nb), dim3(kThreads), 0, ctx->stream, (const float*)x.p,
                           groups, p.stride, partial);
      });
    } else {
      hipLaunchKernelGGL(bn_stats_partial, dim3(p.nb, p.cblocks), dim3(kThreads), 0, ctx->stream,
                         (const float*)x.p, voxels, x.c, x.ld, p.lanes, p.rows, partial);
    }
    MSK_LAUNCH_CHECK(ctx);
  }
  return stats_merge_tail(ctx, partial, p.nb, x.c, p.stride, stats_local, fin);
}

int msk_bn_finalize(msk_ctx* ctx, const float* gathered, int world, double count_per_rank, int C,
                    const float* gamma, const float* beta, float eps, float momentum,
                    float* running_mean, float* running_var, float* save_mean, float* save_invstd,
                    float* scale, float* shift) {
  msk_launch_scope ls(ctx, "bn_finalize");
  hipLaunchKernelGGL(bn_finalize_k, dim3(msk_cdiv(C, 64)), dim3(64), 0, ctx->stream, gathered, world,
                     count_per_rank, C, gamma, beta, eps, momentum, running_mean, running_var, save_mean,
                     save_invstd, scale, shift);
  MSK_LAUNCH_CHECK(ctx);
  return 0;
}

int msk_bn_eval_coeffs(msk_ctx* ctx, int C, const float* gamma, const float* beta, const float* running_mean,
                       const float* running_var, float eps, float* save_mean, float* save_invstd,
                       float* scale, float* shift) {
  msk_launch_scope ls(ctx, "bn_eval_coeffs");
  hipLaunchKernelGGL(bn_eval_coeffs_k, dim3(msk_cdiv(C, 64)), dim3(64), 0, ctx->stream, C, gamma, beta,
                     running_mean, running_var, eps, save_mean, save_invstd, scale, shift);
  MSK_LAUNCH_CHECK(ctx);
  return 0;
}

static int affine_act_fwd_impl(msk_ctx* ctx, msk_tensor x, const float* scale, const float* shift, msk_tensor res,
                               const float* alpha, msk_tensor out, const float* alpha_in, float* out_amax = nullptr,
                               msk_tensor out2 = msk_tensor{}) {
  MSK_REQUIRE(ctx, msk_same_shape(x, out), "x/out shape mismatch");
  MSK_REQUIRE(ctx, (scale == nullptr) == (shift == nullptr), "scale and shift go together");
  if (res.p) MSK_REQUIRE(ctx, res.c > 0 && (res.c == x.c || x.c % res.c == 0), "residual channels must tile");
  const long voxels = msk_voxels(x);
  const EwSel sel = ew_select(PassTensors{x, res, out}, voxels, alpha_in || out2.p);
  msk_launch_scope ls(ctx, "affine_act_fwd");
  if (sel.form != EwForm::CS && out2.p) {
    return msk_fail(ctx, __FILE__, __LINE__, "msk_affine_act_fwd_amax2", "the second output needs the channel-stationary float4 kernel (C / 4 a power of two, aligned tensors)");
  } else if (sel.form == EwForm::D12) {
    const long groups = voxels * x.c / 12;
    d12_ladder(x.c, [&](auto c) {
      hipLaunchKernelGGL(affine_act_fwd_d12_k<decltype(c)::value>, dim3(msk_ew_blocks(groups, ctx->num_cu, g_ew_cap)), dim3(kThreads), 0,
                         ctx->stream, (const float*)x.p, scale, shift, (const float*)res.p, alpha, (float*)out.p, groups,
                         (unsigned*)out_amax);
    });
  } else if (sel.form == EwForm::CS) {
    hipLaunchKernelGGL(affine_act_fwd_cs_k, dim3(msk_ew_blocks(voxels * (x.c / 4) / 2, ctx->num_cu, g_ew_cap)), dim3(kThreads), 0, ctx->stream,
                       (const float*)x.p, x.ld, scale, shift, (const float*)res.p, res.ld, res.c, alpha, (float*)out.p,
                       out.ld, voxels, x.c, sel.cshift, alpha_in, (unsigned*)out_amax, (float*)out2.p, out2.ld);
  } else if (sel.form == EwForm::K4) {
    hipLaunchKernelGGL(affine_act_fwd_k<4>, dim3(msk_ew_blocks(voxels * x.c / 4, ctx->num_cu, g_ew_cap)), dim3(kThreads), 0,
                       ctx->stream, (const float*)x.p, x.ld, scale, shift, (const float*)res.p, res.ld, res.c,
                       alpha, (float*)out.p, out.ld, voxels, x.c, alpha_in, (unsigned*)out_amax);
  } else {
    hipLaunchKernelGGL(affine_act_fwd_k<1>, dim3(msk_ew_blocks(voxels * x.c, ctx->num_cu, g_ew_cap)), dim3(kThreads), 0,
                       ctx->stream, (const float*)x.p, x.ld, scale, shift, (const float*)res.p, res.ld, res.c,
                       alpha, (float*)out.p, out.ld, voxels, x.c, alpha_in, (unsigned*)out_amax);
  }
  MSK_LAUNCH_CHECK(ctx);
  return 0;
}

float* msk_amax_new(msk_ctx* ctx, int n) { return msk_scalar_slots(ctx, n > 0 ? n : 1); }

int msk_affine_act_fwd_amax(msk_ctx* ctx, msk_tensor x, const float* scale, const float* shift, msk_tensor res,
                            const float* alpha, msk_tensor out, float* out_amax) {
  return affine_act_fwd_impl(ctx, x, scale, shift, res, alpha, out, nullptr, out_amax);
}

int msk_affine_act_fwd_amax2(msk_ctx* ctx, msk_tensor x, const float* scale, const float* shift, msk_tensor res,
                             const float* alpha, msk_tensor out, float* out_amax, msk_tensor out2) {
  if (out2.p) MSK_REQUIRE(ctx, msk_same_shape(x, out2) && vec4_ok(out2), "out2 must have x's shape and float4 alignment");
  return affine_act_fwd_impl(ctx, x, scale, shift, res, alpha, out, nullptr, out_amax, out2);
}

int msk_affine_act_join_fwd_amax(msk_ctx* ctx, msk_tensor y, const float* scale, const float* shift, const float* alpha_inner,
                                 msk_tensor res, const float* alpha_outer, msk_tensor out, float* out_amax) {
  MSK_REQUIRE(ctx, scale && shift && alpha_inner && alpha_outer && res.p, "join of a conv -> BN -> PReLU unit with a residual");
  MSK_REQUIRE(ctx, res.c == y.c, "the residual has the unit's channel count");
  return affine_act_fwd_impl(ctx, y, scale, shift, res, alpha_outer, out, alpha_inner, out_amax);
}

int msk_affine_act_fwd(msk_ctx* ctx, msk_tensor x, const float* scale, const float* shift, msk_tensor res,
                       const float* alpha, msk_tensor out) {
  return affine_act_fwd_impl(ctx, x, scale, shift, res, alpha, out, nullptr);
}

int msk_affine_act_join_fwd(msk_ctx* ctx, msk_tensor y, const float* scale, const float* shift, const float* alpha_inner,
                            msk_tensor res, const float* alpha_outer, msk_tensor out) {
  MSK_REQUIRE(ctx, scale && shift && alpha_inner && alpha_outer && res.p, "join of a conv -> BN -> PReLU unit with a residual");
  MSK_REQUIRE(ctx, res.c == y.c, "the residual has the unit's channel count");
  return affine_act_fwd_impl(ctx, y, scale, shift, res, alpha_outer, out, alpha_inner);
}

int msk_affine_act_bwd_reduce(msk_ctx* ctx, msk_tensor x, const float* scale, const float* shift, msk_tensor res,
                              const float* alpha, const float* mean, const float* invstd, msk_tensor dout,
                              float* sums) {
  return msk_affine_act_bwd_reduce_ex(ctx, x, scale, shift, res, alpha, mean, invstd, dout, sums, nullptr);
}

int msk_affine_act_bwd_reduce_ex(msk_ctx* ctx, msk_tensor x, const float* scale, const float* shift, msk_tensor res,
                                 const float* alpha, const float* mean, const float* invstd, msk_tensor dout,
                                 float* sums, float* maxes) {
  return msk_affine_act_bwd_reduce_pg(ctx, x, scale, shift, res, alpha, mean, invstd, dout, sums, maxes, 1, nullptr, nullptr, nullptr);
}

int msk_affine_act_bwd_reduce_pg(msk_ctx* ctx, msk_tensor x, const float* scale, const float* shift, msk_tensor res,
                                 const float* alpha, const float* mean, const float* invstd, msk_tensor dout,
                                 float* sums, float* maxes, int clear_maxes, float* dgamma, float* dbeta, float* dalpha) {
  MSK_REQUIRE(ctx, msk_same_shape(x, dout), "x/dout shape mismatch");
  const long voxels = msk_voxels(x);
  const ReducePlan p = reduce_plan(PassTensors{x, res, dout}, voxels, ctx->num_cu, 1);
  if (maxes) {
    MSK_REQUIRE(ctx, p.form == RedForm::V4, "maxes are produced by the float4 kernel only: channel count and strides multiples of 4, 16-byte aligned tensors");
    if (clear_maxes) MSK_CHECK_HIP(ctx, hipMemsetAsync(maxes, 0, 2 * kWbfAmaxWays * sizeof(float), ctx->stream));
  }
  float* partial = (float*)msk_workspace(ctx, p.bytes(3));
  if (!partial) return -1;
  {
    msk_launch_scope ls(ctx, "affine_act_bwd_reduce");
    if (p.form == RedForm::V4) {
      hipLaunchKernelGGL(affine_act_bwd_reduce_v4_k<0>, dim3(p.nb), dim3(kThreads), 0, ctx->stream,
                         (const float*)x.p, x.ld, scale, shift, (const float*)res.p, res.ld, res.c, alpha, mean, invstd,
                         (const float*)dout.p, dout.ld, voxels, x.c, p.lanes, p.rows, (float*)nullptr, 0, (float*)nullptr, 0, 0,
                         partial, (unsigned*)maxes, (const float*)nullptr);
    } else if (p.form == RedForm::D12) {
// ... 127 lines not shown
  return add_act_bwd_impl(ctx, y, scale, shift, alpha_inner, res, alpha_outer, dout, da, dres, dres_accumulate, dalpha_outer, mean,
                          invstd, unit_sums, maxes, clear_maxes, unit_dgamma, unit_dbeta, unit_dalpha);
}

int msk_affine_act_param_grads(msk_ctx* ctx, int C, const float* sums, float* dgamma, float* dbeta, float* dalpha,
                               int accumulate) {
  msk_launch_scope ls(ctx, "affine_act_param_grads");
  hipLaunchKernelGGL(param_grads_k, dim3(msk_cdiv(C, 64)), dim3(64), 0, ctx->stream, C, sums, dgamma, dbeta,
                     dalpha, accumulate);
  MSK_LAUNCH_CHECK(ctx);
  return 0;
}

int msk_bn_bias_grad(msk_ctx* ctx, int C, const float* sums, const float* scale, float* dbias, int accumulate) {
  MSK_REQUIRE(ctx, sums && scale && dbias, "null pointer");
  msk_launch_scope ls(ctx, "bn_bias_grad");
  hipLaunchKernelGGL(bias_grad_from_sums_k, dim3(msk_cdiv(C, 64)), dim3(64), 0, ctx->stream, C, sums, scale, dbias,
                     accumulate);
  MSK_LAUNCH_CHECK(ctx);
  return 0;
}

int msk_copy_scale(msk_ctx* ctx, msk_tensor src, const float* mask, msk_tensor dst, int accumulate) {
  return msk_copy_scale_amax(ctx, src, mask, dst, accumulate, nullptr);
}

int msk_copy_scale_amax(msk_ctx* ctx, msk_tensor src, const float* mask, msk_tensor dst, int accumulate, float* dst_amax) {
  MSK_REQUIRE(ctx, msk_same_shape(src, dst), "src/dst shape mismatch");
  const long voxels = msk_voxels(src);
  const long vpn = (long)src.d * src.h * src.w;
  msk_launch_scope ls(ctx, "copy_scale");
  if (pass_v4(PassTensors{src, msk_tensor{}, dst})) {
    hipLaunchKernelGGL(copy_scale_k<4>, dim3(msk_ew_blocks(voxels * src.c / 4, ctx->num_cu, g_ew_cap)), dim3(kThreads), 0,
                       ctx->stream, (const float*)src.p, src.ld, mask, (float*)dst.p, dst.ld, voxels, vpn, src.c,
                       accumulate, (unsigned*)dst_amax);
  } else {
    hipLaunchKernelGGL(copy_scale_k<1>, dim3(msk_ew_blocks(voxels * src.c, ctx->num_cu, g_ew_cap)), dim3(kThreads), 0,
                       ctx->stream, (const float*)src.p, src.ld, mask, (float*)dst.p, dst.ld, voxels, vpn, src.c,
                       accumulate, (unsigned*)dst_amax);
  }
  MSK_LAUNCH_CHECK(ctx);
  return 0;
}

int msk_dropout_mask(msk_ctx* ctx, uint64_t seed, uint64_t step, uint32_t site, int count, float p, float* mask) {
  MSK_REQUIRE(ctx, p >= 0.f && p < 1.f, "dropout p must be in [0,1)");
  msk_launch_scope ls(ctx, "dropout_mask");
  hipLaunchKernelGGL(dropout_mask_k, dim3(msk_cdiv(count, 256)), dim3(256), 0, ctx->stream, seed, step, site,
                     count, p, mask);
  MSK_LAUNCH_CHECK(ctx);
  return 0;
}

int msk_channel_sum(msk_ctx* ctx, msk_tensor x, float* out, int accumulate) {
  const long voxels = msk_voxels(x);
  const ReducePlan p = reduce_plan(PassTensors{x}, voxels, ctx->num_cu, 3, false);
  float* partial = (float*)msk_workspace(ctx, p.bytes(1));
  if (!partial) return -1;
  {
    msk_launch_scope ls(ctx, "channel_sum_partial");
    if (p.form == RedForm::D12) {
      const long groups = voxels * x.c / 12;
      const float* const none = nullptr;
      d12_ladder(x.c, [&](auto c) {
        hipLaunchKernelGGL((affine_act_bwd_reduce_d12_k<decltype(c)::value, 1>), dim3(p.nb), dim3(kThreads), 0, ctx->stream,
                           (const float*)x.p, none, none, none, none, none, none, none, groups, p.stride, partial);
      });
    } else {
      hipLaunchKernelGGL(channel_sum_partial_k, dim3(p.nb, p.cblocks), dim3(kThreads), 0, ctx->stream,
                         (const float*)x.p, x.ld, voxels, x.c, p.lanes, p.rows, partial);
    }
    MSK_LAUNCH_CHECK(ctx);
  }
  return sums_merge_tail(ctx, partial, p.nb, x.c, p.stride, 1, out, accumulate);
}

int msk_softmax_c(msk_ctx* ctx, msk_tensor x, msk_tensor out) {
  MSK_REQUIRE(ctx, msk_same_shape(x, out), "x/out shape mismatch");
  const long voxels = msk_voxels(x);
  msk_launch_scope ls(ctx, "softmax_c");
  hipLaunchKernelGGL(softmax_c_k, dim3(msk_ew_blocks(voxels, ctx->num_cu, g_ew_cap)), dim3(kThreads), 0, ctx->stream, (const float*)x.p, x.ld,
                     voxels, x.c, (float*)out.p, out.ld);
  MSK_LAUNCH_CHECK(ctx);
  return 0;
}

int msk_argmax_c(msk_ctx* ctx, msk_tensor x, int32_t* out) {
  const long voxels = msk_voxels(x);
  msk_launch_scope ls(ctx, "argmax_c");
  hipLaunchKernelGGL(argmax_k, dim3(msk_ew_blocks(voxels, ctx->num_cu, g_ew_cap)), dim3(kThreads), 0, ctx->stream,
                     (const float*)x.p, x.ld, voxels, x.c, out);
  MSK_LAUNCH_CHECK(ctx);
  return 0;
}

}

namespace {
__global__ void __launch_bounds__(kThreads)
absmax_k(const float* __restrict__ x, int ld, int C, long voxels, unsigned* __restrict__ slot) {
  float m = 0.f;
  if (ld == C && (voxels * C) % 4 == 0 && (((uintptr_t)x) & 15) == 0) {
    const float4* p = reinterpret_cast<const float4*>(x);
    const long total = voxels * C / 4, stride = (long)gridDim.x * blockDim.x;
    auto fold = [&](const float4 q) { m = fmaxf(fmaxf(m, fmaxf(fabsf(q.x), fabsf(q.y))), fmaxf(fabsf(q.z), fabsf(q.w))); };
    long i = (long)blockIdx.x * blockDim.x + threadIdx.x;
// ... 187 lines not shown
```

medicalseg_amd/models/vnet.py:

```python
from __future__ import annotations

import os

import numpy as np

from .. import nn
from ..cvlibs import manager
from ..device import Tensor, get_device, to_tensor
from ..nn import AddAct, ConvBNAct, copy_scale

DENSE_TWIN = os.environ.get("MSEGK_DENSE_TWIN", "1") != "0"
SPLIT_CONCAT_GRAD = os.environ.get("MSEGK_SPLIT_CONCAT_GRAD", "1") != "0"


class LUConv(nn.Layer):

    def __init__(self, nchan, elu):
        super(LUConv, self).__init__()
        self.relu1 = nn.ELU() if elu else nn.PReLU(nchan)
        self.conv1 = nn.Conv3D(nchan, nchan, kernel_size=5, padding=2)
        self.bn1 = nn.BatchNorm3D(nchan)
        self._unit = ConvBNAct(self.conv1, self.bn1, self.relu1)

    def forward(self, x):
# ... 11 lines not shown
def _run_ops(ops, x, res):
    ops = list(ops)
    out = x
    for op in ops[:-1]:
        out = op(out)
    if not ops:
        return out, None
    last = ops[-1]
    if isinstance(last, LUConv) and _join_fusable(out, res):
        out = last._unit.forward(out, defer_act=True)
        return out, (last._unit if last._unit.deferred else None)
    return last(out), None


def _make_nConv(nchan, depth, elu):
    return nn.Sequential(*[LUConv(nchan, elu) for _ in range(depth)])


class InputTransition(nn.Layer):

    def __init__(self, in_channels, elu):
        super(InputTransition, self).__init__()
        self.num_features = 16
        self.in_channels = in_channels
        if self.num_features % in_channels:
            raise ValueError("in_channels must divide 16 (x.tile in the reference, vnet.py:76-78)")
        self.conv1 = nn.Conv3D(self.in_channels, self.num_features, kernel_size=5, padding=2)
        self.bn1 = nn.BatchNorm3D(self.num_features)
        self.relu1 = nn.ELU() if elu else nn.PReLU(self.num_features)
        self._unit = ConvBNAct(self.conv1, self.bn1, self.relu1)

    def forward(self, x, out=None, out2=None):
        return self._unit.forward(x, res=x, out=out, out2=out2)

    def backward(self, dout):
        self._unit.backward(dout, need_dx=False, res_needs_grad=False)


class DownTransition(nn.Layer):

    def __init__(self, inChans, nConvs, elu, dropout=False, downsample_stride=(2, 2, 2), kernel=(2, 2, 2)):
        super(DownTransition, self).__init__()
        outChans = 2 * inChans
        self.if_dropout = dropout
        self.down_conv = nn.Conv3D(inChans, outChans, kernel_size=kernel, stride=downsample_stride)
        self.bn1 = nn.BatchNorm3D(outChans)
        self.relu1 = nn.ELU() if elu else nn.PReLU(outChans)
        self.relu2 = nn.ELU() if elu else nn.PReLU(outChans)
        self.dropout = nn.Dropout3D()
        self.ops = _make_nConv(outChans, nConvs, elu)
        self._down = ConvBNAct(self.down_conv, self.bn1, self.relu1)
        self._join = AddAct(self.relu2)

    def forward(self, x, out=None):
        down = self._down.forward(x)
        self._mask = self.dropout.make_mask(down) if self.if_dropout else None
        if self._mask is not None:
            t = down.empty_like()
            copy_scale(down, self._mask, t)
        else:
            t = down
        self._dropped = t
        self._t_down = down
        t, unit = _run_ops(self.ops, t, down)
        self._t_ops = t
        return self._join.forward(t, down, unit=unit, out=out)

    def backward(self, dout):
        down = self._t_down
        ops = list(self.ops)
        self._join.backward(dout, share_b=bool(ops) and self._mask is None and ops[0]._unit.x is down)
        for op in reversed(ops):
            g = op._unit.out.grad
            op.backward(g)
        nn.materialize_grad(down)
        if self._mask is not None:
            copy_scale(self._dropped.grad, self._mask, down.grad, accumulate=True)
        self._down.backward(down.grad)


class UpTransition(nn.Layer):

    def __init__(self, inChans, outChans, nConvs, elu, dropout=False, dropout2=False,
                 upsample_stride_size=(2, 2, 2), kernel=(2, 2, 2)):
        super(UpTransition, self).__init__()
        self.up_conv = nn.Conv3DTranspose(inChans, outChans // 2, kernel_size=kernel, stride=upsample_stride_size)
        self.bn1 = nn.BatchNorm3D(outChans // 2)
        self.relu1 = nn.ELU() if elu else nn.PReLU(outChans // 2)
        self.relu2 = nn.ELU() if elu else nn.PReLU(outChans)
        self.if_dropout = dropout
        self.if_dropout2 = dropout2
        self.dropout1 = nn.Dropout3D()
        self.dropout2 = nn.Dropout3D()
        self.ops = _make_nConv(outChans, nConvs, elu)
        self.outChans = outChans
        self._up = ConvBNAct(self.up_conv, self.bn1, self.relu1)
        self._join = AddAct(self.relu2)

    def reserve_concat(self, dev, n, dims):
        self._reserved = None
        if self.if_dropout2 or os.environ.get("MSEGK_ZERO_COPY_SKIP", "1") == "0":
            return None
        half = self.outChans // 2
        xcat = Tensor.empty(dev, n, dims[0], dims[1], dims[2], self.outChans)
        if nn.PRODUCER_AMAX:
            xcat.amax = dev.amax_new()
        self._reserved = xcat
        self._reserved_skip = xcat.channel_slice(half, self.outChans)
        return self._reserved_skip

    def forward(self, x, skipx):
        dev = x.dev
        self._x, self._skip = x, skipx
        self._m1 = self.dropout1.make_mask(x) if self.if_dropout else None
        self._m2 = self.dropout2.make_mask(skipx) if self.if_dropout2 else None
        xin = x
        if self._m1 is not None:
            xin = x.empty_like()
            copy_scale(x, self._m1, xin)
        self._xin = xin
        half = self.outChans // 2
        od, oh, ow = self.up_conv.out_dims(xin)
        if (od, oh, ow) != (skipx.d, skipx.h, skipx.w) or skipx.c != self.outChans - half:
            raise ValueError(f"skip connection shape {skipx.shape} does not match the up-sampled "
                             f"({x.n}, {half}, {od}, {oh}, {ow})")
        res = getattr(self, "_reserved", None)
        self._reserved = None
        self._skip_in_place = (res is not None and self._m2 is None and skipx.ld == res.ld and
                               skipx.ptr == res.ptr + 4 * half and res.gen == dev.arena.gen)
        if self._skip_in_place:
            xcat, s_skip = res, skipx
        else:
            xcat = Tensor.empty(dev, x.n, od, oh, ow, self.outChans)
            if nn.PRODUCER_AMAX:
                xcat.amax = dev.amax_new()
            s_skip = xcat.channel_slice(half, self.outChans)
        s_up = xcat.channel_slice(0, half)
        self._up.forward(xin, out=s_up)
        if not self._skip_in_place:
            copy_scale(skipx, self._m2, s_skip)
        if xcat.amax is None or s_up.amax != xcat.amax or s_skip.amax != xcat.amax:
            xcat.amax = None
        self._xcat = xcat
        out, unit = _run_ops(self.ops, xcat, xcat)
        return self._join.forward(out, xcat, unit=unit)

    def join_for_consumer(self):
        ops = list(self.ops)
        return self._join, bool(ops) and ops[0]._unit.x is self._xcat

    def backward(self, dout):
        xcat, half = self._xcat, self.outChans // 2
        ops = list(self.ops)
        self._join.backward(dout, share_b=bool(ops) and ops[0]._unit.x is xcat)
        g_lo = g_hi = None
        skip = self._skip
        first = ops[0]._unit if ops else None
        if (first is not None and SPLIT_CONCAT_GRAD and self._skip_in_place and skip.grad is None and half * 4 < 128 and self._m1 is None):
            dev = xcat.dev
            g_lo = Tensor.empty(dev, xcat.n, xcat.d, xcat.h, xcat.w, half)
            g_hi = Tensor.empty(dev, xcat.n, xcat.d, xcat.h, xcat.w, half)
            first.dx_split = (g_lo, g_hi)
        if first is not None:
            first.dx_split_done = False
        for op in reversed(ops):
            op.backward(op._unit.out.grad)
        nn.materialize_grad(xcat)
        gcat = xcat.grad
        split_done = g_lo is not None and getattr(first, "dx_split_done", False)
        if first is not None:
            first.dx_split = None
        if split_done:
            skip.grad = g_hi
        elif self._skip_in_place and skip.grad is None:
            skip.grad = gcat.channel_slice(half, self.outChans)
        else:
            sg = skip.ensure_grad()
            copy_scale(gcat.channel_slice(half, self.outChans), self._m2, sg, accumulate=skip.grad_written)
        skip.grad_written = True
        self._up.backward(g_lo if split_done else gcat.channel_slice(0, half))
        if self._m1 is not None:
            x = self._x
            xg = x.ensure_grad()
            copy_scale(self._xin.grad, self._m1, xg, accumulate=x.grad_written)
            x.grad_written = True


class OutputTransition(nn.Layer):

    def __init__(self, in_channels, num_classes, elu):
        super(OutputTransition, self).__init__()
        self.conv1 = nn.Conv3D(in_channels, num_classes, kernel_size=5, padding=2)
        self.bn1 = nn.BatchNorm3D(num_classes)
        self.conv2 = nn.Conv3D(num_classes, num_classes, kernel_size=1)
        self.relu1 = nn.ELU() if elu else nn.PReLU(num_classes)
        self._unit = ConvBNAct(self.conv1, self.bn1, self.relu1)

    def forward(self, x):
# ... 22 lines not shown
        self.down_tr64 = DownTransition(32, 2, elu, downsample_stride=stride_size[1], kernel=kernel_size[1])
        self.down_tr128 = DownTransition(64, 3, elu, dropout=True, downsample_stride=stride_size[2],
                                         kernel=kernel_size[2])
        self.down_tr256 = DownTransition(128, 2, elu, dropout=True, downsample_stride=stride_size[3],
                                         kernel=kernel_size[3])
        self.up_tr256 = UpTransition(256, 256, 2, elu, dropout=True, dropout2=True,
                                     upsample_stride_size=stride_size[3], kernel=kernel_size[3])
        self.up_tr128 = UpTransition(256, 128, 2, elu, dropout=True, dropout2=True,
                                     upsample_stride_size=stride_size[2], kernel=kernel_size[2])
        self.up_tr64 = UpTransition(128, 64, 1, elu, upsample_stride_size=stride_size[1], kernel=kernel_size[1])
        self.up_tr32 = UpTransition(64, 32, 1, elu, upsample_stride_size=stride_size[0], kernel=kernel_size[0])
        self.out_tr = OutputTransition(32, num_classes, elu)

        self.pretrained = pretrained
        self._post_backward_hooks = []
        self._grad_ready_hooks = []
        self._build()
        self.init_weight()

    def _build(self):
        dev = get_device()
        params, frozen = [], []
        for name, p in self.named_parameters():
            p.name = name
            (frozen if getattr(p, "frozen", False) else params).append(p)
        bufs = []
        for name, p in self.named_buffers():
            p.name = name
            bufs.append(p)
        self.arena = nn.ParamArena(dev, params, with_grad=True)
        self.buffer_arena = nn.ParamArena(dev, bufs, with_grad=False)
        self.frozen_arena = nn.ParamArena(dev, frozen, with_grad=False) if frozen else None
        self.dev = dev

    def init_weight(self):
        if self.pretrained is not None:
            from ..utils import utils
            utils.load_entire_model(self, self.pretrained)

    def dropout_layers(self):
        return {"down_tr128": self.down_tr128.dropout, "down_tr256": self.down_tr256.dropout,
                "up_tr256.x": self.up_tr256.dropout1, "up_tr256.skip": self.up_tr256.dropout2,
                "up_tr128.x": self.up_tr128.dropout1, "up_tr128.skip": self.up_tr128.dropout2}

    def set_dropout_masks(self, masks):
        for site, layer in self.dropout_layers().items():
            if masks is None:
                layer.injected, layer.enabled = None, True
            elif site in masks and masks[site] is not None:
                layer.injected, layer.enabled = np.asarray(masks[site], dtype=np.float32), True
            else:
                layer.injected, layer.enabled = None, False

    def forward(self, x):
        if not isinstance(x, Tensor):
            x = to_tensor(x, self.dev)
        if x.c != self.in_channels:
            raise ValueError(f"VNet expects {self.in_channels} input channel(s), got {x.c}")
        self.dev.arena.reset()
        if self.training:
            nn.Dropout3D.step += 1
        slot = self.up_tr32.reserve_concat(self.dev, x.n, (x.d, x.h, x.w))
        twin = None
        if slot is not None and DENSE_TWIN and self.training and slot.c * 4 < 128 and not isinstance(self.in_tr.relu1, nn.ELU):
            twin = Tensor.empty(self.dev, x.n, x.d, x.h, x.w, slot.c)
        out16 = self.in_tr(x, out=slot, out2=twin)
        self._out16_twin = twin
        out32 = self.down_tr32(twin if twin is not None else out16,
                               out=self.up_tr64.reserve_concat(self.dev, x.n, self.down_tr32.down_conv.out_dims(out16)))
        out64 = self.down_tr64(out32)
        out128 = self.down_tr128(out64)
        out256 = self.down_tr256(out128)
        out = self.up_tr256(out256, out128)
        out = self.up_tr128(out, out64)
        out = self.up_tr64(out, out32)
        self._feat = self.up_tr32(out, out16)
        logits = self.out_tr(self._feat)
        logits.producer = self
        self._acts = (out16, out32, out64, out128, out256)
        return [logits, ]

    def backward(self, dlogits: Tensor):
        out16, out32, out64, out128, out256 = self._acts
        twin = getattr(self, "_out16_twin", None)

        def share_twin_grad():
            if twin is not None and out16.grad is not None:
                twin.grad, twin.grad_written = out16.grad, True
        self.out_tr.backward(dlogits, join=self.up_tr32.join_for_consumer())
        self._grads_ready(self.out_tr)
        for block, dout in (
                            (self.up_tr32, lambda: self._feat.grad),
                            (self.up_tr64, lambda: self.up_tr32._x.grad),
                            (self.up_tr128, lambda: self.up_tr64._x.grad),
                            (self.up_tr256, lambda: self.up_tr128._x.grad),
                            (self.down_tr256, lambda: out256.grad),
                            (self.down_tr128, lambda: out128.grad),
                            (self.down_tr64, lambda: out64.grad),
                            (self.down_tr32, lambda: out32.grad),
                            (self.in_tr, lambda: out16.grad)):
            block.backward(dout())
            if block is self.up_tr32:
                share_twin_grad()
            self._grads_ready(block)
        for hook in self._post_backward_hooks:
            hook(self)

    def _grads_ready(self, block):
        for hook in self._grad_ready_hooks:
            hook(self, block)

    def test(self):
        np.random.seed(1)
        a = np.random.rand(1, self.in_channels, 32, 32, 32)
        out = self.forward(a.astype("float32"))[0]
        assert out.shape == (1, self.num_classes, 32, 32, 32)
        print("out", out.numpy().mean(), a.mean())
        print("Vnet test is complete")
```

medicalseg_amd/models/vnet_deepsup.py:

```python
from __future__ import annotations

import ctypes as C

import numpy as np

from .. import nn
from ..cvlibs import manager
from ..device import Tensor, get_device, to_tensor
from .vnet import DownTransition, InputTransition, OutputTransition, UpTransition, VNet


def interpolate_trilinear(x: Tensor, size) -> Tensor:
    d, h, w = (int(v) for v in size)
    out = Tensor.empty(x.dev, x.n, d, h, w, x.c)
    x.dev.call("msk_interp_trilinear_fwd", x.msk(), out.msk())
    return out


def interpolate_trilinear_backward(dout: Tensor, x: Tensor):
    dev = x.dev
    g = x.ensure_grad()
    need = C.c_size_t(0)
    dev.call("msk_interp_scratch_bytes", g.msk(), dout.msk(), C.byref(need))
    scratch = dev.arena.alloc(max(int(need.value), 16))
# ... 1 lines not shown
             C.c_size_t(int(need.value)))
    x.grad_written = True


@manager.MODELS.add_component
class VNetDeepSup(VNet):

    num_outputs = 4

    def __init__(self, elu=False, in_channels=1, num_classes=4, pretrained=None,
                 kernel_size=((2, 2, 2), (2, 2, 2), (2, 2, 2), (2, 2, 2)),
                 stride_size=((2, 2, 2), (2, 2, 2), (2, 2, 2), (2, 2, 2)), native_heads=False):
        nn.Layer.__init__(self)
        self.native_heads = bool(native_heads)
        self.best_loss = 1000000
        self.num_classes = num_classes
        self.in_channels = in_channels

        self.in_tr = InputTransition(in_channels, elu=elu)
        self.down_tr32 = DownTransition(16, 1, elu, downsample_stride=stride_size[0], kernel=kernel_size[0])
        self.down_tr64 = DownTransition(32, 2, elu, downsample_stride=stride_size[1], kernel=kernel_size[1])
        self.down_tr128 = DownTransition(64, 3, elu, dropout=True, downsample_stride=stride_size[2],
                                         kernel=kernel_size[2])
        self.down_tr256 = DownTransition(128, 2, elu, dropout=True, downsample_stride=stride_size[3],
                                         kernel=kernel_size[3])
        self.up_tr256 = UpTransition(256, 256, 2, elu, dropout=True, dropout2=True,
                                     upsample_stride_size=stride_size[3], kernel=kernel_size[3])
        self.up_tr128 = UpTransition(256, 128, 2, elu, dropout=True, dropout2=True,
                                     upsample_stride_size=stride_size[2], kernel=kernel_size[2])
        self.up_tr64 = UpTransition(128, 64, 1, elu, upsample_stride_size=stride_size[1], kernel=kernel_size[1])
        self.up_tr32 = UpTransition(64, 32, 1, elu, upsample_stride_size=stride_size[0], kernel=kernel_size[0])
        self.out_tr32 = OutputTransition(32, num_classes, elu)
        self.out_tr64 = nn.Conv3D(64, num_classes, kernel_size=3, padding=1)
        self.out_tr128 = nn.Conv3D(128, num_classes, kernel_size=3, padding=1)
        self.out_tr256 = nn.Conv3D(256, num_classes, kernel_size=3, padding=1)
        self.out_tr_all = OutputTransition(4 * num_classes, num_classes, elu)
        for p in self.out_tr_all.parameters():
            p.frozen = True

        self.pretrained = pretrained
        self._post_backward_hooks = []
        self._grad_ready_hooks = []
        self._build()
        self.init_weight()

    def forward(self, x):
        if not isinstance(x, Tensor):
            x = to_tensor(x, self.dev)
        if x.c != self.in_channels:
            raise ValueError(f"VNetDeepSup expects {self.in_channels} input channel(s), got {x.c}")
        self.dev.arena.reset()
        if self.training:
            nn.Dropout3D.step += 1
        size = (x.d, x.h, x.w)
        out16 = self.in_tr(x, out=self.up_tr32.reserve_concat(self.dev, x.n, (x.d, x.h, x.w)))
        out32 = self.down_tr32(out16, out=self.up_tr64.reserve_concat(self.dev, x.n, self.down_tr32.down_conv.out_dims(out16)))
        out64 = self.down_tr64(out32)
        out128 = self.down_tr128(out64)
        out256 = self.down_tr256(out128)
        native = self.native_heads
        heads_on = self.training or not native

        def head(conv, feat):
            if not heads_on:
                return None, None
            h = conv.run_forward(feat)
            return h, (h if native else interpolate_trilinear(h, size))

        u256 = self.up_tr256(out256, out128)
        h1, d1 = head(self.out_tr256, u256)
        u128 = self.up_tr128(u256, out64)
        h2, d2 = head(self.out_tr128, u128)
        u64 = self.up_tr64(u128, out32)
        h3, d3 = head(self.out_tr64, u64)
        self._feat = self.up_tr32(u64, out16)
        out = self.out_tr32(self._feat)
        self._acts = (out16, out32, out64, out128, out256)
        self._ups = (u256, u128, u64)
        self._heads = (h1, h2, h3)
        outs = [out, d1, d2, d3] if heads_on else [out]
        for i, t in enumerate(outs):
            t.producer, t.out_index = self, i
        if native and heads_on:
            extents = tuple((h.d, h.h, h.w) for h in self._heads)
            for i, h in enumerate(self._heads):
                h.native_head = (extents, i)
        return outs

    def _head_backward(self, conv, feat: Tensor, head: Tensor, dresized):
        if dresized is None:
            return
        if self.native_heads:
            conv.run_backward(feat, dresized, need_dx=True)
        else:
            interpolate_trilinear_backward(dresized, head)
            conv.run_backward(feat, head.grad, need_dx=True)
        self._grads_ready(conv)

    def backward(self, dlogits):
        if isinstance(dlogits, Tensor):
            dlogits = [dlogits, None, None, None]
        dout, dd1, dd2, dd3 = dlogits
        u256, u128, u64 = self._ups
        h1, h2, h3 = self._heads
        def run(block, dy):
            block.backward(dy)
# ... 28 lines not shown
```

medicalseg_amd/nn.py:

```python
from __future__ import annotations

import ctypes as C
import os
import warnings
from collections import OrderedDict

import numpy as np

from . import _lib
from ._lib import NULL_TENSOR, MskBnFin, MskConvDesc, MskError
from .device import Tensor, get_device
from .optimizer import ClipGradByGlobalNorm, ClipGradByNorm, ClipGradByValue

BN_EPS = 1e-5
BN_MOMENTUM = 0.9


def _triple(v):
    if isinstance(v, (list, tuple)):
        if len(v) != 3:
            raise ValueError(f"expected 3 values, got {v}")
        return tuple(int(i) for i in v)
    return (int(v),) * 3

# ... 316 lines not shown
            base = dev.small(total)
            o = 0
            s = {"world": W}
            for name, cnt in (("stats", 2 * Cn), ("gathered", W * 2 * Cn), ("scale", Cn), ("shift", Cn),
                              ("mean", Cn), ("invstd", Cn), ("sums", 4 * Cn), ("sums_total", 3 * Cn), ("maxes", 128)):
                s[name] = base + 4 * o
                o += cnt
            self._scratch = s
        return self._scratch


class SyncBatchNorm(BatchNorm3D):
    @staticmethod
    def convert_sync_batchnorm(layer):
        return layer


class PReLU(Layer):

    def __init__(self, num_parameters=1, init=0.25):
        super().__init__()
        self.num_parameters = int(num_parameters)
        self._weight = Parameter(np.full(num_parameters, init))


class ELU(Layer):

    def __init__(self, alpha=1.0):
        super().__init__()
        self.alpha = float(alpha)


def _act_alpha(act):
    return act._weight.ptr if isinstance(act, PReLU) else None


def _act_alpha_grad(act):
    return act._weight.grad_ptr if isinstance(act, PReLU) else None


class Dropout3D(Layer):

    _site_counter = 0
    seed = 0
    step = 0

    def __init__(self, p=0.5):
        super().__init__()
        self.p = float(p)
        Dropout3D._site_counter += 1
        self.site = Dropout3D._site_counter
        self.injected = None
        self.enabled = True

    def make_mask(self, x: Tensor):
        if not self.training or not self.enabled or self.p == 0.0:
            return None
        dev = x.dev
        cnt = x.n * x.c
        ptr = dev.arena.alloc(cnt * 4)
        if self.injected is not None:
            m = np.ascontiguousarray(self.injected, dtype=np.float32)
            if m.shape != (x.n, x.c):
                raise ValueError(f"injected dropout mask must be [{x.n},{x.c}], got {m.shape}")
            dev.h2d(ptr, m)
        else:
            dev.call("msk_dropout_mask", C.c_uint64(Dropout3D.seed), C.c_uint64(Dropout3D.step),
                     C.c_uint32(self.site | (dev.rank << 16)), cnt, C.c_float(self.p), C.c_void_p(ptr))
        return ptr


_FUSED_INFERENCE = {"on": False, "epoch": 0}


class fused_inference:

    def __enter__(self):
        self._prev = _FUSED_INFERENCE["on"]
        _FUSED_INFERENCE["on"] = True
        if not self._prev:
            _FUSED_INFERENCE["epoch"] += 1
        return self

    def __exit__(self, *exc):
        _FUSED_INFERENCE["on"] = self._prev
        return False


def _fp(ptr):
    return C.c_void_p(ptr) if ptr else None


PRODUCER_AMAX = os.environ.get("MSEGK_PRODUCER_AMAX", "1") != "0"


def _amax_for(out: Tensor):
    if not PRODUCER_AMAX:
        return None
    if out.amax is None:
        out.amax = out.dev.amax_new()
    return C.c_void_p(out.amax)


FUSE_SMALL = os.environ.get("MSEGK_FUSE_SMALL", "1") != "0"


KS_STATS = os.environ.get("MSEGK_KS_STATS", "1") != "0"
FUSE_BN_BACKWARD = os.environ.get("MSEGK_BWD_FUSE", "1") != "0"
FUSE_BN_BACKWARD_C1 = os.environ.get("MSEGK_BWD_FUSE_C1", "1") != "0"
FUSE_BN_BACKWARD_T = os.environ.get("MSEGK_BWD_FUSE_T", "0") == "1"


SHARE_JOIN_GRAD = os.environ.get("MSEGK_SHARE_JOIN_GRAD", "1") != "0"


def materialize_grad(t: Tensor):
    src = getattr(t, "grad_from", None)
    if src is None:
        return
    t.grad_from = None
    g = t.ensure_grad()
    src.dev.call("msk_copy_scale", src.msk(), None, g.msk(), 1 if t.grad_written else 0)
    g.amax = None
    t.grad_written = True


class ConvBNAct:

    def __init__(self, conv, bn: BatchNorm3D, act: PReLU | None):
        self.conv, self.bn, self.act = conv, bn, act

    def _forward_folded(self, x: Tensor, out: Tensor | None) -> Tensor:
        dev, conv, bn = x.dev, self.conv, self.bn
        if x.c != conv.cin:
            raise ValueError(f"Conv3D expects {conv.cin} input channels, got {x.c}")
        if getattr(self, "_fold_epoch", None) != _FUSED_INFERENCE["epoch"]:
            if not hasattr(self, "_fold_w"):
                self._fold_w = dev.malloc(conv.weight.size * 4)
                self._fold_b = dev.malloc(conv.cout * 4)
            sc, Cn = bn.scratch(dev), bn.num_features
            dev.call("msk_bn_eval_coeffs", Cn, _fp(bn.weight.ptr), _fp(bn.bias.ptr), _fp(bn._mean.ptr),
                     _fp(bn._variance.ptr), C.c_float(bn.epsilon), _fp(sc["mean"]), _fp(sc["invstd"]),
                     _fp(sc["scale"]), _fp(sc["shift"]))
            dev.call("msk_conv_fold_bn", _fp(conv.weight.ptr), _fp(conv.bias.ptr), _fp(sc["scale"]), _fp(sc["shift"]),
                     conv.cout, C.c_long(conv.weight.size // conv.cout), _fp(self._fold_w), _fp(self._fold_b))
            self._fold_epoch = _FUSED_INFERENCE["epoch"]
        if out is None:
            od, oh, ow = conv.out_dims(x)
            out = Tensor.empty(dev, x.n, od, oh, ow, conv.cout)
        alpha = _act_alpha(self.act)
        dev.call("msk_conv3d_fwd_act", conv.desc(), x.msk(), _fp(self._fold_w), _fp(self._fold_b), _fp(alpha), out.msk())
        out.amax = None
        self.x, self.res, self.y, self.out, self.bn_mode = x, None, None, out, 3
        return out

    def forward(self, x: Tensor, res: Tensor | None = None, out: Tensor | None = None, defer_act=False, out2: Tensor | None = None) -> Tensor:
        dev = x.dev
        self.deferred = False
        if (_FUSED_INFERENCE["on"] and not self.bn.training and res is None and type(self.conv) is Conv3D
                and (self.act is None or isinstance(self.act, PReLU))):
            return self._forward_folded(x, out)
        self.x, self.res = x, res
        bn, sc = self.bn, self.bn.scratch(dev)
        Cn = bn.num_features
        fin = None
        multi = (dev.world > 1 or BatchNorm3D.force_collectives) and BatchNorm3D.sync and not BatchNorm3D.dry_run
        if bn.training and FUSE_SMALL and not multi:
            od, oh, ow = self.conv.out_dims(x)
            fin = MskBnFin(bn.weight.ptr, bn.bias.ptr, bn.epsilon, bn.momentum, float(x.n * od * oh * ow), bn._mean.ptr,
                           bn._variance.ptr, sc["mean"], sc["invstd"], sc["scale"], sc["shift"])
        if bn.training and type(self.conv) is Conv3D:
            y = self.conv.run_forward(x, stats_ptr=sc["stats"], keep_xform=True, fin=fin)
        elif bn.training and type(self.conv) is Conv3DTranspose and KS_STATS:
            conv = self.conv
            if x.c != conv.cin:
                raise ValueError(f"Conv3DTranspose expects {conv.cin} input channels, got {x.c}")
            od, oh, ow = conv.out_dims(x)
            y = Tensor.empty(dev, x.n, od, oh, ow, conv.cout)
            _count_flops(conv, x.n, x.d * x.h * x.w, 1)
            dev.call("msk_convT3d_fwd_ex", conv.desc(), x.msk(), _fp(conv.weight.ptr), _fp(conv.bias.ptr), y.msk(), _fp(sc["stats"]),
                     C.byref(fin) if fin is not None else None)
        else:
            y = self.conv.run_forward(x)
            if bn.training:
                if fin is not None:
                    dev.call("msk_bn_stats_fin", y.msk(), _fp(sc["stats"]), C.byref(fin))
                else:
                    dev.call("msk_bn_stats", y.msk(), _fp(sc["stats"]))
        self.y = y
        if bn.training:
            if fin is None:
                gathered, nstat = sc["stats"], 1
                if multi:
                    dev.call("msk_dp_allgather", _fp(sc["stats"]), _fp(sc["gathered"]), C.c_size_t(2 * Cn))
                    gathered, nstat = sc["gathered"], dev.world
                dev.call("msk_bn_finalize", _fp(gathered), nstat, C.c_double(y.voxels), Cn, _fp(bn.weight.ptr),
                         _fp(bn.bias.ptr), C.c_float(bn.epsilon), C.c_float(bn.momentum), _fp(bn._mean.ptr),
                         _fp(bn._variance.ptr), _fp(sc["mean"]), _fp(sc["invstd"]), _fp(sc["scale"]), _fp(sc["shift"]))
            self.bn_mode = 1
        else:
            dev.call("msk_bn_eval_coeffs", Cn, _fp(bn.weight.ptr), _fp(bn.bias.ptr), _fp(bn._mean.ptr),
                     _fp(bn._variance.ptr), C.c_float(bn.epsilon), _fp(sc["mean"]), _fp(sc["invstd"]),
                     _fp(sc["scale"]), _fp(sc["shift"]))
            self.bn_mode = 2
        if out is None:
            out = y.empty_like()
        alpha = _act_alpha(self.act)
        if defer_act and res is None and alpha is not None:
            self.deferred = True
        else:
            if isinstance(self.act, ELU):
                dev.call("msk_affine_act_fwd", y.msk(), _fp(sc["scale"]), _fp(sc["shift"]),
                         res.msk() if res is not None else NULL_TENSOR, _fp(alpha), out.msk())
                dev.call("msk_elu_fwd", out.msk(), C.c_float(self.act.alpha), out.msk())
                out.amax = None
            elif out2 is not None:
                dev.call("msk_affine_act_fwd_amax2", y.msk(), _fp(sc["scale"]), _fp(sc["shift"]),
                         res.msk() if res is not None else NULL_TENSOR, _fp(alpha), out.msk(), _amax_for(out), out2.msk())
                out2.amax = out.amax
            else:
                dev.call("msk_affine_act_fwd_amax", y.msk(), _fp(sc["scale"]), _fp(sc["shift"]),
                         res.msk() if res is not None else NULL_TENSOR, _fp(alpha), out.msk(), _amax_for(out))
        self.out = out
        return out

    def backward(self, dout: Tensor, need_dx=True, res_needs_grad=True, join=None):
        if self.bn_mode == 3:
            raise RuntimeError("backward through a forward pass run under nn.fused_inference() (BN folded into the "
                               "convolution: no pre-activation tensor was kept)")
        dev = dout.dev
        bn, sc = self.bn, self.bn.scratch(dev)
        Cn = bn.num_features
        y, res = self.y, self.res
        alpha = _act_alpha(self.act)
        if isinstance(self.act, ELU):
            g = Tensor.empty(dev, dout.n, dout.d, dout.h, dout.w, dout.c)
            dev.call("msk_elu_bwd", self.out.msk(), dout.msk(), C.c_float(self.act.alpha), g.msk(), 0)
            dout = g
        resm = res.msk() if res is not None else NULL_TENSOR
        fuse = (FUSE_BN_BACKWARD and type(self.conv) is Conv3D and res is None and self.bn_mode == 1 and need_dx
                and self.conv.cin == self.conv.cout)
        if not fuse:
            materialize_grad(self.x)
        want_maxes = fuse and Cn % 4 == 0 and y.ld % 4 == 0 and dout.ld % 4 == 0 and y.ptr % 16 == 0 and dout.ptr % 16 == 0
        pg_done = False
        maxes = sc["maxes"]
        if getattr(self, "presummed", False):
            self.presummed = False
            want_maxes = fuse
            pg_done = getattr(self, "presummed_pg", False)
            maxes = getattr(self, "presummed_maxes", None) or sc["maxes"]
        elif want_maxes and FUSE_SMALL:
            maxes = dev.amax_new(2)
            dev.call("msk_affine_act_bwd_reduce_pg", y.msk(), _fp(sc["scale"]), _fp(sc["shift"]), resm, _fp(alpha),
                     _fp(sc["mean"]), _fp(sc["invstd"]), dout.msk(), _fp(sc["sums"]), _fp(maxes), 0,
                     _fp(bn.weight.grad_ptr), _fp(bn.bias.grad_ptr), _fp(_act_alpha_grad(self.act)))
            pg_done = True
        elif want_maxes:
            dev.call("msk_affine_act_bwd_reduce_ex", y.msk(), _fp(sc["scale"]), _fp(sc["shift"]), resm, _fp(alpha),
                     _fp(sc["mean"]), _fp(sc["invstd"]), dout.msk(), _fp(sc["sums"]), _fp(sc["maxes"]))
        elif FUSE_SMALL:
            dev.call("msk_affine_act_bwd_reduce_pg", y.msk(), _fp(sc["scale"]), _fp(sc["shift"]), resm, _fp(alpha),
                     _fp(sc["mean"]), _fp(sc["invstd"]), dout.msk(), _fp(sc["sums"]), None, 0,
                     _fp(bn.weight.grad_ptr), _fp(bn.bias.grad_ptr), _fp(_act_alpha_grad(self.act)))
            pg_done = True
        else:
            dev.call("msk_affine_act_bwd_reduce", y.msk(), _fp(sc["scale"]), _fp(sc["shift"]), resm, _fp(alpha),
                     _fp(sc["mean"]), _fp(sc["invstd"]), dout.msk(), _fp(sc["sums"]))
# ... 57 lines not shown
                         split[0].msk(), split[1].msk(), C.byref(done))
                self.dx_split_done = bool(done.value)
            else:
                dev.call("msk_conv3d_bwd_bnact", conv.desc(), x.msk(), _fp(conv.weight.ptr), y.msk(), _fp(sc["scale"]),
                         _fp(sc["shift"]), _fp(alpha), _fp(sc["mean"]), _fp(sc["invstd"]), _fp(bn.weight.ptr), dout.msk(),
                         _fp(sums_total), C.c_double(m_total), dy.msk(), dx.msk(), 1 if x.grad_written else 0,
                         _fp(conv.weight.grad_ptr), 1, _fp(xfp), _fp(ybuf), _fp(maxes) if want_maxes else None)
            x.grad_written = True
            conv._xform = None
            self.dy = dy if ybuf is None else None
            return
        if (FUSE_BN_BACKWARD and FUSE_BN_BACKWARD_T and type(self.conv) is Conv3DTranspose and self.bn_mode == 1 and need_dx
                and res is None and not isinstance(self.act, ELU) and self.conv.cout <= 16):
            conv, x = self.conv, self.x
            dx = x.ensure_grad()
            rc = dev.lib.msk_convT3d_bwd_bnact(dev.ctx, conv.desc(), x.msk(), _fp(conv.weight.ptr), y.msk(), _fp(sc["scale"]),
                                               _fp(sc["shift"]), _fp(alpha), _fp(sc["mean"]), _fp(sc["invstd"]), dout.msk(),
                                               _fp(sums_total), C.c_double(m_total), dy.msk(), dx.msk(),
                                               1 if x.grad_written else 0, _fp(conv.weight.grad_ptr), 1)
            if rc < 0:
                raise MskError(f"msk_convT3d_bwd_bnact failed: {_lib.last_error(dev.ctx)}")
            if rc == 0:
                _count_flops(conv, x.n, x.d * x.h * x.w, 2)
                x.grad_written = True
                self.dy = dy
                return
        if (join is not None and res is None and need_dx and type(self.conv) is Conv3D and self.bn_mode == 1
                and not isinstance(self.act, ELU) and self.conv.s == (1, 1, 1)
                and join[0].backward_in_dgrad(self, join[1], dout, dy, sums_total, m_total)):
            self.dy = dy
            return
        dres = NULL_TENSOR
        dres_acc = 0
        if res is not None and res_needs_grad and res.c == y.c:
            g = res.ensure_grad()
            dres, dres_acc = g.msk(), 1 if res.grad_written else 0
            res.grad_written = True
        dya = _amax_for(dy) if type(self.conv) is Conv3D and self.conv.s == (1, 1, 1) else None
        dev.call("msk_affine_act_bwd_apply_amax", y.msk(), _fp(sc["scale"]), _fp(sc["shift"]), resm, _fp(alpha),
                 _fp(sc["mean"]), _fp(sc["invstd"]), _fp(bn.weight.ptr), dout.msk(), _fp(sums_total),
                 C.c_double(m_total), self.bn_mode, dy.msk(), dres, dres_acc, dya)
        self.dy = dy
        if self.bn_mode == 2:
            dev.call("msk_bn_bias_grad", Cn, _fp(sc["sums"]), _fp(sc["scale"]), _fp(self.conv.bias.grad_ptr), 1)
        self.conv.run_backward(self.x, dy, need_dx=need_dx, bias_grad=False)


class AddAct:

    def __init__(self, act: PReLU):
        self.act = act
        self._sums = None

    def forward(self, a: Tensor, b: Tensor, unit: "ConvBNAct | None" = None, out: Tensor | None = None) -> Tensor:
        self.a, self.b = a, b
        self._bwd_done = False
        self.unit = unit if (unit is not None and getattr(unit, "deferred", False)) else None
        if out is None:
            out = a.empty_like()
        if isinstance(self.act, ELU):
            a.dev.call("msk_affine_act_fwd", a.msk(), None, None, b.msk(), None, out.msk())
            a.dev.call("msk_elu_fwd", out.msk(), C.c_float(self.act.alpha), out.msk())
            out.amax = None
            self.out = out
            return out
        if self.unit is not None:
            u, sc = self.unit, self.unit.bn.scratch(a.dev)
            a.dev.call("msk_affine_act_join_fwd_amax", u.y.msk(), _fp(sc["scale"]), _fp(sc["shift"]), _fp(u.act._weight.ptr),
                       b.msk(), _fp(self.act._weight.ptr), out.msk(), _amax_for(out))
        else:
            a.dev.call("msk_affine_act_fwd_amax", a.msk(), None, None, b.msk(), _fp(self.act._weight.ptr), out.msk(),
                       _amax_for(out))
        self.out = out
        return out

    def backward_in_dgrad(self, consumer: "ConvBNAct", share_b, dout: Tensor, dy: Tensor, sums_total, m_total) -> bool:
        dev = dout.dev
        a, b, u = self.a, self.b, getattr(self, "unit", None)
        x, conv = consumer.x, consumer.conv
        if getattr(dev.lib.msk_conv3d_bwd_bnact_join, "missing", False):
            warnings.warn(f"{_lib.LIB_PATH} does not export msk_conv3d_bwd_bnact_join: the residual join behind the output block "
                          "runs as separate kernels; rebuild with ./build.sh", RuntimeWarning)
            return False
        if (u is None or not FUSE_SMALL or isinstance(self.act, ELU)
                or getattr(self, "out", None) is not x or x.grad is not None or getattr(x, "grad_from", None) is not None
                or a.grad_written or b.grad_written or a.c % 4):
            return False
        ga, gb = a.ensure_grad(), b.ensure_grad()
        share_b = bool(share_b and SHARE_JOIN_GRAD and ga.ld == gb.ld)
        if not all(t.ld % 4 == 0 and t.ptr % 16 == 0 for t in (a, b, ga, gb, u.y)):
            return False
        sc, usc = consumer.bn.scratch(dev), u.bn.scratch(dev)
        y = consumer.y
        xf = getattr(conv, "_xform", None)
        xfp = xf[0] if (xf is not None and xf[1] == x.ptr and xf[2] == dev.arena.gen) else None
        dya = _amax_for(dy)
        xa = x.amax if (x.amax and PRODUCER_AMAX and xfp is None) else None
        mx = dev.amax_new(2)
        rc = dev.lib.msk_conv3d_bwd_bnact_join(
            dev.ctx, conv.desc(), x.msk(), _fp(conv.weight.ptr), y.msk(), _fp(sc["scale"]), _fp(sc["shift"]),
            _fp(_act_alpha(consumer.act)), _fp(sc["mean"]), _fp(sc["invstd"]), _fp(consumer.bn.weight.ptr), dout.msk(),
            _fp(sums_total), C.c_double(m_total), dy.msk(), dya, _fp(conv.weight.grad_ptr), 1, _fp(xfp), _fp(xa),
            u.y.msk(), _fp(usc["scale"]), _fp(usc["shift"]), _fp(u.act._weight.ptr), b.msk(), _fp(self.act._weight.ptr),
            _fp(usc["mean"]), _fp(usc["invstd"]), ga.msk(), 0, NULL_TENSOR if share_b else gb.msk(), 0,
            _fp(self.act._weight.grad_ptr), _fp(usc["sums"]), _fp(mx), 0,
            _fp(u.bn.weight.grad_ptr), _fp(u.bn.bias.grad_ptr), _fp(u.act._weight.grad_ptr))
        if rc < 0:
            raise MskError(f"msk_conv3d_bwd_bnact_join failed: {_lib.last_error(dev.ctx)}")
        if rc != 0:
            return False
        _count_flops(conv, x.n, dy.d * dy.h * dy.w, 2)
        conv._xform = None
        u.presummed, u.presummed_pg, u.presummed_maxes = True, True, mx
        a.grad_written = True
        if share_b:
            b.grad_from = ga
        else:
            b.grad_written = True
        self._bwd_done = True
        return True

    def backward(self, dout: Tensor, share_b=False):
# ... 61 lines not shown
```

Measured before the change: 246.7 million.

## Fuse dropout into activation epilogue, batch mask draws, fuse BN stats into conv

Adds elementwise kernels that write the activation output and also a dropout-scaled second copy into a reserved skip buffer, so the separate dropout copy pass over the tensor is skipped. All dropout masks for a step are drawn in one batched launch instead of one launch per site. The kernel-split forward convolution also gains a statistics variant that computes per-block Welford partials of BN mean and variance in its epilogue and merges them, removing a separate stats pass. This adds complexity in buffer reservation and new code paths, and idle waves are kept alive in stats mode so they can join the block-level reduction.

```diff
diff --git a/include/msegk.h b/include/msegk.h
--- a/include/msegk.h
+++ b/include/msegk.h
@@ -171,6 +171,12 @@
                        msk_tensor res, const float* alpha, msk_tensor out);
 int msk_affine_act_fwd_amax2(msk_ctx* ctx, msk_tensor x, const float* scale, const float* shift, msk_tensor res,
                              const float* alpha, msk_tensor out, float* out_amax , msk_tensor out2);
+int msk_affine_act_fwd_amax2s(msk_ctx* ctx, msk_tensor x, const float* scale, const float* shift, msk_tensor res,
+                              const float* alpha, msk_tensor out, float* out_amax , msk_tensor out2,
+                              const float* out2_scale , float* out2_amax );
+int msk_affine_act_join_fwd_amax2s(msk_ctx* ctx, msk_tensor y, const float* scale, const float* shift, const float* alpha_inner,
+                                   msk_tensor res, const float* alpha_outer, msk_tensor out, float* out_amax ,
+                                   msk_tensor out2, const float* out2_scale , float* out2_amax );
 int msk_affine_act_bwd_reduce(msk_ctx* ctx, msk_tensor x, const float* scale, const float* shift,
                               msk_tensor res, const float* alpha, const float* mean,
                               const float* invstd, msk_tensor dout, float* sums);
@@ -193,6 +199,14 @@
 int msk_copy_scale(msk_ctx* ctx, msk_tensor src, const float* mask, msk_tensor dst, int accumulate);
 int msk_dropout_mask(msk_ctx* ctx, uint64_t seed, uint64_t step, uint32_t site, int count,
                      float p, float* mask);
+#define MSK_DROPOUT_MAX_SITES 8
+typedef struct {
+  uint32_t site;
+  int32_t count;
+  float p;
+  float* mask;
+} msk_dropout_site;
+int msk_dropout_masks(msk_ctx* ctx, uint64_t seed, uint64_t step, const msk_dropout_site* sites, int n);
 int msk_channel_sum(msk_ctx* ctx, msk_tensor x, float* out, int accumulate);
 int msk_argmax_c(msk_ctx* ctx, msk_tensor x, int32_t* out);
 int msk_softmax_c(msk_ctx* ctx, msk_tensor x, msk_tensor out);
diff --git a/medicalseg_amd/_lib.py b/medicalseg_amd/_lib.py
--- a/medicalseg_amd/_lib.py
+++ b/medicalseg_amd/_lib.py
@@ -27,6 +27,12 @@
                 ("count", C.c_double), ("running_mean", C.c_void_p), ("running_var", C.c_void_p),
                 ("save_mean", C.c_void_p), ("save_invstd", C.c_void_p), ("scale", C.c_void_p), ("shift", C.c_void_p)]
 
+
+class MskDropoutSite(C.Structure):
+    _fields_ = [("site", C.c_uint32), ("count", C.c_int32), ("p", C.c_float), ("mask", C.c_void_p)]
+
+
+DROPOUT_MAX_SITES = 8
 
 NULL_TENSOR = MskTensor(None, 0, 0, 0, 0, 0, 0)
 
@@ -83,6 +89,8 @@
     "msk_affine_act_fwd_amax": (_i, [_vp, _T, _vp, _vp, _T, _vp, _T, _vp]),
     "msk_affine_act_fwd_amax2": (_i, [_vp, _T, _vp, _vp, _T, _vp, _T, _vp, _T]),
     "msk_affine_act_join_fwd_amax": (_i, [_vp, _T, _vp, _vp, _vp, _T, _vp, _T, _vp]),
+    "msk_affine_act_fwd_amax2s": (_i, [_vp, _T, _vp, _vp, _T, _vp, _T, _vp, _T, _vp, _vp]),
+    "msk_affine_act_join_fwd_amax2s": (_i, [_vp, _T, _vp, _vp, _vp, _T, _vp, _T, _vp, _T, _vp, _vp]),
     "msk_copy_scale_amax": (_i, [_vp, _T, _vp, _T, _i, _vp]),
     "msk_conv3d_bwd_bnact_bytes": (_sz, [_vp, _CD, _T, _T]),
     "msk_conv3d_bwd_bnact": (_i, [_vp, _CD, _T, _vp, _T, _vp, _vp, _vp, _vp, _vp, _vp, _T, _vp, _d, _T, _T, _i, _vp, _i, _vp, _vp, _vp]),
@@ -118,6 +126,7 @@
     "msk_bn_bias_grad": (_i, [_vp, _i, _vp, _vp, _vp, _i]),
     "msk_copy_scale": (_i, [_vp, _T, _vp, _T, _i]),
     "msk_dropout_mask": (_i, [_vp, _u64, _u64, _u32, _i, _f, _vp]),
+    "msk_dropout_masks": (_i, [_vp, _u64, _u64, _vp, _i]),
     "msk_channel_sum": (_i, [_vp, _T, _vp, _i]),
     "msk_argmax_c": (_i, [_vp, _T, _vp]),
     "msk_softmax_c": (_i, [_vp, _T, _T]),
diff --git a/medicalseg_amd/csrc/msk_common.h b/medicalseg_amd/csrc/msk_common.h
--- a/medicalseg_amd/csrc/msk_common.h
+++ b/medicalseg_amd/csrc/msk_common.h
@@ -130,6 +130,7 @@
   int dst_split = 1;
   int wgrad_reduce_rows = 1;
   int ks_stats = 1;
+  int dropout_fuse = 1;
   int ks_lds = 1;
   int ks_nr_max = 4;
   int wgrad_lds_pad = 0;
diff --git a/medicalseg_amd/csrc/msk_conv_ksfwd.hip b/medicalseg_amd/csrc/msk_conv_ksfwd.hip
--- a/medicalseg_amd/csrc/msk_conv_ksfwd.hip
+++ b/medicalseg_amd/csrc/msk_conv_ksfwd.hip
@@ -1,4 +1,5 @@
 #include "msk_conv.h"
+#include "msk_wbf.h"
 #ifdef KS_PROBE_NOMFMA
 #define __builtin_amdgcn_mfma_f32_32x32x2f32(a_, b_, c_, x_, y_, z_) ks_probe_keep((a_), (b_), (c_))
 #define __builtin_amdgcn_mfma_f32_16x16x4f32(a_, b_, c_, x_, y_, z_) ks_probe_keep((a_), (b_), (c_))
@@ -20,14 +21,66 @@
   float invM;
 };
 
-template <int NR, int KB, bool FUSE = false>
+struct KsRec { float n, mean, m2; };
+__device__ __forceinline__ KsRec ksrec_merge(KsRec a, KsRec b) {
+  if (b.n == 0.f) return a;
+  if (a.n == 0.f) return b;
+  KsRec r;
+  r.n = a.n + b.n;
+  const float d = b.mean - a.mean, f = b.n / r.n;
+  r.mean = a.mean + d * f;
+  r.m2 = a.m2 + b.m2 + d * d * a.n * f;
+  return r;
+}
+template <int NR>
+__device__ __forceinline__ void ks_stats_tail(const f32x16 (&val)[NR], bool vok, float nvalid, int nt0, int CN, float* __restrict__ partial) {
+  __shared__ float shr[4][32 * NR][3];
+  const int tid = threadIdx.x, wave = tid >> 6, lane = tid & 63, li = lane & 31, lh = lane >> 5;
+#pragma unroll
+  for (int r = 0; r < NR; ++r)
+#pragma unroll
+    for (int i = 0; i < 16; ++i) {
+      const float x = val[r][i];
+      const float k0 = __builtin_bit_cast(float, __builtin_amdgcn_readlane(__builtin_bit_cast(int, x), 0));
+      const float k1 = __builtin_bit_cast(float, __builtin_amdgcn_readlane(__builtin_bit_cast(int, x), 32));
+      const float K = lh ? k1 : k0;
+      const float d = vok ? x - K : 0.f;
+      float s1 = d, s2 = d * d;
+#pragma unroll
+      for (int o = 1; o < 32; o <<= 1) {
+        s1 += __shfl_xor(s1, o, 64);
+        s2 += __shfl_xor(s2, o, 64);
+      }
+      if (li == 0) {
+        float* p = shr[wave][r * 32 + 8 * (i >> 2) + 4 * lh + (i & 3)];
+        p[0] = nvalid;
+        p[1] = nvalid > 0.f ? K + s1 / nvalid : 0.f;
+        p[2] = nvalid > 0.f ? fmaxf(s2 - s1 * s1 / nvalid, 0.f) : 0.f;
+      }
+    }
+  __syncthreads();
+  const int cn = nt0 * 32 + tid;
+  if (tid < 32 * NR && cn < CN) {
+    KsRec t = {shr[0][tid][0], shr[0][tid][1], shr[0][tid][2]};
+#pragma unroll
+    for (int w = 1; w < 4; ++w) t = ksrec_merge(t, KsRec{shr[w][tid][0], shr[w][tid][1], shr[w][tid][2]});
+    float* o = partial + ((long)blockIdx.x * CN + cn) * 3;
+    o[0] = t.n; o[1] = t.mean; o[2] = t.m2;
+  }
+}
+
+template <int NR, int KB, bool FUSE = false, bool STATS = false>
 __global__ void __launch_bounds__(256, FUSE ? 2 : (NR == 1 ? 4 : (NR == 2 ? 4 : 2)))
-gconv_ks_fwd_k(GConv g, const float4* __restrict__ wm, int KC, int npad, unsigned src_bytes, KsBnBwd bn) {
+gconv_ks_fwd_k(GConv g, const float4* __restrict__ wm, int KC, int npad, unsigned src_bytes, KsBnBwd bn, float* __restrict__ stat_partial) {
+  static_assert(!(FUSE && STATS), "the statistics form is a forward convolution");
   const int tid = threadIdx.x;
   const int wave = tid >> 6, lane = tid & 63, li = lane & 31, lh = lane >> 5;
   const long M = (long)g.N * g.DD * g.DH * g.DW;
   const long m = ((long)blockIdx.x * 4 + wave) * 32 + li;
-  if (((long)blockIdx.x * 4 + wave) * 32 >= M) return;
+  const long wm0 = ((long)blockIdx.x * 4 + wave) * 32;
+  if constexpr (!STATS) {
+    if (wm0 >= M) return;
+  }
   const bool mok = m < M;
   unsigned ow, oh, od, n;
   {
@@ -137,7 +190,9 @@
     load(xa, wa);
     if (t0 + KB < T) compute(xb, wb);
   }
-  if (!mok) return;
+  if constexpr (!STATS) {
+    if (!mok) return;
+  }
 
   float* orow = g.dst + m * g.dld;
 #pragma unroll
@@ -147,7 +202,7 @@
 #pragma unroll
     for (int q = 0; q < 4; ++q) {
       const int cn = (nt0 + r) * 32 + 8 * q + 4 * lh;
-      ok[q] = cn < g.CN;
+      ok[q] = mok && cn < g.CN;
       old[q] = (g.accumulate && ok[q]) ? *reinterpret_cast<const float4*>(orow + cn) : make_float4(0.f, 0.f, 0.f, 0.f);
     }
 #pragma unroll
@@ -161,17 +216,25 @@
         v.z = acc[r][4 * q + 2] + bv.z + old[q].z;
         v.w = acc[r][4 * q + 3] + bv.w + old[q].w;
         *reinterpret_cast<float4*>(orow + cn) = v;
-      }
-    }
+        if constexpr (STATS) {
+          acc[r][4 * q + 0] = v.x; acc[r][4 * q + 1] = v.y; acc[r][4 * q + 2] = v.z; acc[r][4 * q + 3] = v.w;
+        }
+      }
+    }
+  }
+  if constexpr (STATS) {
+    const long left = M - wm0;
+    ks_stats_tail<NR>(acc, mok, left <= 0 ? 0.f : (left < 32 ? (float)left : 32.f), nt0, g.CN, stat_partial);
   }
 }
 
 #ifndef KS_DBG
 #define KS_DBG 0
 #endif
-template <int NR, int CK, bool FUSE>
+template <int NR, int CK, bool FUSE, bool STATS = false>
 __global__ void __launch_bounds__(256, 3)
-gconv_ks_lds_k(GConv g, const float4* __restrict__ wm, int npad, KsBnBwd bn, int runs) {
+gconv_ks_lds_k(GConv g, const float4* __restrict__ wm, int npad, KsBnBwd bn, int runs, float* __restrict__ stat_partial) {
+  static_assert(!(FUSE && STATS), "the statistics form is a forward convolution");
   constexpr int KC = CK / 8, QV = CK / 4;
   constexpr int PP = 2 * CK * 4 + 16;
   constexpr int ROWB = 32 * PP;
@@ -179,8 +242,12 @@
   __shared__ __attribute__((aligned(16))) char lds[4 * 2 * ROWB];
   const int tid = threadIdx.x;
   const int wave = __builtin_amdgcn_readfirstlane(tid >> 6), lane = tid & 63, li = lane & 31, lh = lane >> 5;
-  const int rid = blockIdx.x * 4 + wave;
-  if (rid >= runs) return;
+  const int rid0 = blockIdx.x * 4 + wave;
+  const bool live = rid0 < runs;
+  if constexpr (!STATS) {
+    if (!live) return;
+  }
+  const int rid = live ? rid0 : runs - 1;
   char* reg = lds + wave * 2 * ROWB;
   const int rpr = g.DW / 32;
   int t = rid / rpr;
@@ -300,9 +367,13 @@
       v.y = acc[r][4 * q + 1] + bv.y + old[q].y;
       v.z = acc[r][4 * q + 2] + bv.z + old[q].z;
       v.w = acc[r][4 * q + 3] + bv.w + old[q].w;
-      if (!(KS_DBG & 4) || v.x == 12345.678f) *reinterpret_cast<float4*>(orow + cn) = v;
-    }
-  }
+      if ((!(KS_DBG & 4) || v.x == 12345.678f) && live) *reinterpret_cast<float4*>(orow + cn) = v;
+      if constexpr (STATS) {
+        acc[r][4 * q + 0] = v.x; acc[r][4 * q + 1] = v.y; acc[r][4 * q + 2] = v.z; acc[r][4 * q + 3] = v.w;
+      }
+    }
+  }
+  if constexpr (STATS) ks_stats_tail<NR>(acc, live, live ? 32.f : 0.f, nt0, g.CN, stat_partial);
 }
 
 template <int NR, int KB, bool PAIR = false>
@@ -490,6 +561,7 @@
   const float* wm = msk_pack_weights_get(ctx, w_canon, A, B, taps, swap, 0, g.kd, g.kh, g.kw, 1, g.CK, g.CN, KC, npad);
   if (!wm) return -1;
   const int ntn = npad / 32;
+  const bool stats = g.stats != nullptr && !g.stats_ps && !g.accumulate && !bnp && !g.prelu && ctx->ks_stats == 1;
   if (ctx->ks_lds && g.kd == 2 && g.kh == 2 && g.kw == 2 && g.sd == 2 && g.sh == 2 && g.sw == 2 && g.SD == 2 * g.DD && g.SH == 2 * g.DH &&
       g.SW == 2 * g.DW && g.DW % 32 == 0 && (g.CK == 8 || g.CK == 16) && g.CN % 32 == 0 && (!g.bias || ((uintptr_t)g.bias) % 16 == 0)) {
     const int runs = (int)(M / 32);
@@ -501,19 +573,31 @@
                g.accumulate, NRl);
       tag = msk_intern_tag(ctx, buf);
     }
-    msk_launch_scope ls(ctx, tag);
     const dim3 grid((unsigned)((runs + 3) / 4), ntn / NRl);
-    const float4* w4 = reinterpret_cast<const float4*>(wm);
-    const KsBnBwd bnv = bnp ? *bnp : KsBnBwd{};
+    float* sp = nullptr;
+    if (stats) {
+      sp = (float*)msk_workspace(ctx, (size_t)grid.x * g.CN * 3 * sizeof(float));
+      if (!sp) return -1;
+    }
+    {
+      msk_launch_scope ls(ctx, tag);
+      const float4* w4 = reinterpret_cast<const float4*>(wm);
+      const KsBnBwd bnv = bnp ? *bnp : KsBnBwd{};
 #define KS_LDS(NR_, CK_) \
-    do { \
-      if (bnp) hipLaunchKernelGGL((gconv_ks_lds_k<NR_, CK_, true>), grid, dim3(256), 0, ctx->stream, g, w4, npad, bnv, runs); \
-      else hipLaunchKernelGGL((gconv_ks_lds_k<NR_, CK_, false>), grid, dim3(256), 0, ctx->stream, g, w4, npad, bnv, runs); \
-    } while (0)
-    if (g.CK == 16) { if (NRl == 2) KS_LDS(2, 16); else KS_LDS(1, 16); }
-    else { if (NRl == 2) KS_LDS(2, 8); else KS_LDS(1, 8); }
+      do { \
+        if (bnp) hipLaunchKernelGGL((gconv_ks_lds_k<NR_, CK_, true>), grid, dim3(256), 0, ctx->stream, g, w4, npad, bnv, runs, sp); \
+        else if (stats) hipLaunchKernelGGL((gconv_ks_lds_k<NR_, CK_, false, true>), grid, dim3(256), 0, ctx->stream, g, w4, npad, bnv, runs, sp); \
+        else hipLaunchKernelGGL((gconv_ks_lds_k<NR_, CK_, false>), grid, dim3(256), 0, ctx->stream, g, w4, npad, bnv, runs, sp); \
+      } while (0)
+      if (g.CK == 16) { if (NRl == 2) KS_LDS(2, 16); else KS_LDS(1, 16); }
+      else { if (NRl == 2) KS_LDS(2, 8); else KS_LDS(1, 8); }
 #undef KS_LDS
-    MSK_LAUNCH_CHECK(ctx);
+      MSK_LAUNCH_CHECK(ctx);
+    }
+    if (stats) {
+      if (msk_bn_stats_merge(ctx, sp, (int)grid.x, g.CN, g.stats, g.fin) != 0) return -1;
+      ctx->stats_fused = true;
+    }
     return 1;
   }
   const long mtiles = (M + 127) / 128;
@@ -528,22 +612,35 @@
              g.DW, g.sld, g.dld, g.accumulate, NR);
     tag = msk_intern_tag(ctx, buf);
   }
-  msk_launch_scope ls(ctx, tag);
   dim3 grid((unsigned)mtiles, ntn / NR);
-  const float4* w4 = reinterpret_cast<const float4*>(wm);
-  switch (NR) {
-    case 4:
-      hipLaunchKernelGGL((gconv_ks_fwd_k<4, 2>), grid, dim3(256), 0, ctx->stream, g, w4, KC, npad, (unsigned)sbytes, KsBnBwd{});
-      break;
-    case 2:
-      if (bnp) hipLaunchKernelGGL((gconv_ks_fwd_k<2, 2, true>), grid, dim3(256), 0, ctx->stream, g, w4, KC, npad, (unsigned)sbytes, *bnp);
-      else hipLaunchKernelGGL((gconv_ks_fwd_k<2, 2>), grid, dim3(256), 0, ctx->stream, g, w4, KC, npad, (unsigned)sbytes, KsBnBwd{});
-      break;
-    default:
-      if (bnp) hipLaunchKernelGGL((gconv_ks_fwd_k<1, 2, true>), grid, dim3(256), 0, ctx->stream, g, w4, KC, npad, (unsigned)sbytes, *bnp);
-      else hipLaunchKernelGGL((gconv_ks_fwd_k<1, 4>), grid, dim3(256), 0, ctx->stream, g, w4, KC, npad, (unsigned)sbytes, KsBnBwd{});
-      break;
-  }
-  MSK_LAUNCH_CHECK(ctx);
+  float* sp = nullptr;
+  if (stats) {
+    sp = (float*)msk_workspace(ctx, (size_t)mtiles * g.CN * 3 * sizeof(float));
+    if (!sp) return -1;
+  }
+  {
+    msk_launch_scope ls(ctx, tag);
+    const float4* w4 = reinterpret_cast<const float4*>(wm);
+#define KS_FWD(NR_, KB_, KBF_) \
+    do { \
+      if (bnp) hipLaunchKernelGGL((gconv_ks_fwd_k<NR_, KBF_, true>), grid, dim3(256), 0, ctx->stream, g, w4, KC, npad, (unsigned)sbytes, *bnp, sp); \
+      else if (stats) hipLaunchKernelGGL((gconv_ks_fwd_k<NR_, KB_, false, true>), grid, dim3(256), 0, ctx->stream, g, w4, KC, npad, (unsigned)sbytes, KsBnBwd{}, sp); \
+      else hipLaunchKernelGGL((gconv_ks_fwd_k<NR_, KB_>), grid, dim3(256), 0, ctx->stream, g, w4, KC, npad, (unsigned)sbytes, KsBnBwd{}, sp); \
+    } while (0)
+    switch (NR) {
+      case 4:
+        if (stats) hipLaunchKernelGGL((gconv_ks_fwd_k<4, 2, false, true>), grid, dim3(256), 0, ctx->stream, g, w4, KC, npad, (unsigned)sbytes, KsBnBwd{}, sp);
+        else hipLaunchKernelGGL((gconv_ks_fwd_k<4, 2>), grid, dim3(256), 0, ctx->stream, g, w4, KC, npad, (unsigned)sbytes, KsBnBwd{}, sp);
+        break;
+      case 2: KS_FWD(2, 2, 2); break;
+      default: KS_FWD(1, 4, 2); break;
+    }
+#undef KS_FWD
+    MSK_LAUNCH_CHECK(ctx);
+  }
+  if (stats) {
+    if (msk_bn_stats_merge(ctx, sp, (int)mtiles, g.CN, g.stats, g.fin) != 0) return -1;
+    ctx->stats_fused = true;
+  }
   return 1;
 }
diff --git a/medicalseg_amd/csrc/msk_ctx.hip b/medicalseg_amd/csrc/msk_ctx.hip
--- a/medicalseg_amd/csrc/msk_ctx.hip
+++ b/medicalseg_amd/csrc/msk_ctx.hip
@@ -411,6 +411,7 @@
   else if (strcmp(key, "world") == 0) *value = ctx->world;
   else if (strcmp(key, "rank") == 0) *value = ctx->rank;
   else if (strcmp(key, "num_cu") == 0) *value = ctx->num_cu;
+  else if (strcmp(key, "dropout_fuse") == 0) *value = ctx->dropout_fuse;
   else if (strcmp(key, "scalar_ring_served") == 0) *value = (int)(ctx->scalar_served & 0x3FFFFFFF);
   else if (strcmp(key, "scalar_ring_served_side") == 0) *value = (int)(ctx->scalar_served_side & 0x3FFFFFFF);
   else if (msk_get_ew_option(key, value)) {}
@@ -542,6 +543,10 @@
   }
   if (strcmp(key, "ks_stats") == 0) {
     ctx->ks_stats = value;
+    return 0;
+  }
+  if (strcmp(key, "dropout_fuse") == 0) {
+    ctx->dropout_fuse = value;
     return 0;
   }
   if (strcmp(key, "ks_lds") == 0) {
diff --git a/medicalseg_amd/csrc/msk_elementwise.hip b/medicalseg_amd/csrc/msk_elementwise.hip
--- a/medicalseg_amd/csrc/msk_elementwise.hip
+++ b/medicalseg_amd/csrc/msk_elementwise.hip
@@ -342,12 +342,19 @@
   if (out_amax) block_atomic_max(out_amax, mx);
 }
 
+struct EwOut2Scale {
+  const float* scale;
+  long vox_per_n;
+  unsigned* amax;
+};
+template <bool S2 = false>
 __global__ void EW_BOUNDS
 affine_act_fwd_cs_k(const float* __restrict__ x, int ldx, const float* __restrict__ scale,
                     const float* __restrict__ shift, const float* __restrict__ res, int ldr, int cres,
                     const float* __restrict__ alpha, float* __restrict__ out, int ldo, long voxels, int C, int cshift,
-                    const float* __restrict__ alpha_in, unsigned* __restrict__ out_amax, float* __restrict__ out2, int ldo2) {
-  float mx = 0.f;
+                    const float* __restrict__ alpha_in, unsigned* __restrict__ out_amax, float* __restrict__ out2, int ldo2,
+                    EwOut2Scale s2 = EwOut2Scale{}) {
+  float mx = 0.f, mx2 = 0.f;
   const long g = (long)blockIdx.x * kThreads + threadIdx.x;
   const int c = (int)(g & ((C >> 2) - 1)) * 4;
   const long vstride = ((long)gridDim.x * kThreads) >> cshift;
@@ -381,7 +388,17 @@
     }
     mx = fmaxf(fmaxf(mx, fmaxf(fabsf(o[0]), fabsf(o[1]))), fmaxf(fabsf(o[2]), fabsf(o[3])));
     *reinterpret_cast<float4*>(out + v * ldo + c) = make_float4(o[0], o[1], o[2], o[3]);
-    if (out2) *reinterpret_cast<float4*>(out2 + v * ldo2 + c) = make_float4(o[0], o[1], o[2], o[3]);
+    if constexpr (S2) {
+      if (s2.scale) {
+        const float* m = s2.scale + (v / s2.vox_per_n) * C + c;
+#pragma unroll
+        for (int j = 0; j < 4; ++j) o[j] *= m[j];
+      }
+      mx2 = fmaxf(fmaxf(mx2, fmaxf(fabsf(o[0]), fabsf(o[1]))), fmaxf(fabsf(o[2]), fabsf(o[3])));
+      *reinterpret_cast<float4*>(out2 + v * ldo2 + c) = make_float4(o[0], o[1], o[2], o[3]);
+    } else {
+      if (out2) *reinterpret_cast<float4*>(out2 + v * ldo2 + c) = make_float4(o[0], o[1], o[2], o[3]);
+    }
   };
   long v = g >> cshift;
   for (; v + vstride < voxels; v += 2 * vstride) {
@@ -393,6 +410,9 @@
   }
   if (v < voxels) body(v, *reinterpret_cast<const float4*>(x + v * ldx + c), load_res(v));
   if (out_amax) block_atomic_max(out_amax, mx);
+  if constexpr (S2) {
+    if (s2.amax) block_atomic_max(s2.amax, mx2);
+  }
 }
 
 __global__ void __launch_bounds__(kThreads)
@@ -838,6 +858,18 @@
   float u = (float)(h >> 40) * (1.0f / 16777216.0f);
   mask[i] = u >= p ? 1.0f / (1.0f - p) : 0.f;
 }
+struct DropoutSites {
+  msk_dropout_site e[MSK_DROPOUT_MAX_SITES];
+};
+__global__ void dropout_masks_k(uint64_t seed, uint64_t step, DropoutSites s) {
+  const msk_dropout_site e = s.e[blockIdx.y];
+  int i = blockIdx.x * blockDim.x + threadIdx.x;
+  if (i >= e.count) return;
+  uint64_t h = splitmix64(seed ^ splitmix64(step * 0x100000001B3ull + e.site));
+  h = splitmix64(h + (uint64_t)i);
+  float u = (float)(h >> 40) * (1.0f / 16777216.0f);
+  e.mask[i] = u >= e.p ? 1.0f / (1.0f - e.p) : 0.f;
+}
 
 __global__ void argmax_k(const float* __restrict__ x, int ld, long voxels, int C, int32_t* __restrict__ out) {
   for (long v = (long)blockIdx.x * blockDim.x + threadIdx.x; v < voxels; v += (long)gridDim.x * blockDim.x) {
@@ -1312,12 +1344,21 @@
 
 static int affine_act_fwd_impl(msk_ctx* ctx, msk_tensor x, const float* scale, const float* shift, msk_tensor res,
                                const float* alpha, msk_tensor out, const float* alpha_in, float* out_amax = nullptr,
-                               msk_tensor out2 = msk_tensor{}) {
+                               msk_tensor out2 = msk_tensor{}, const EwOut2Scale* s2 = nullptr) {
   MSK_REQUIRE(ctx, msk_same_shape(x, out), "x/out shape mismatch");
   MSK_REQUIRE(ctx, (scale == nullptr) == (shift == nullptr), "scale and shift go together");
   if (res.p) MSK_REQUIRE(ctx, res.c > 0 && (res.c == x.c || x.c % res.c == 0), "residual channels must tile");
   const long voxels = msk_voxels(x);
   const EwSel sel = ew_select(PassTensors{x, res, out}, voxels, alpha_in || out2.p);
+  if (s2) {
+    if (sel.form != EwForm::CS || !ctx->dropout_fuse) return 1;
+    msk_launch_scope ls(ctx, "affine_act_fwd");
+    hipLaunchKernelGGL(affine_act_fwd_cs_k<true>, dim3(msk_ew_blocks(voxels * (x.c / 4) / 2, ctx->num_cu, g_ew_cap)), dim3(kThreads), 0, ctx->stream,
+                       (const float*)x.p, x.ld, scale, shift, (const float*)res.p, res.ld, res.c, alpha, (float*)out.p,
+                       out.ld, voxels, x.c, sel.cshift, alpha_in, (unsigned*)out_amax, (float*)out2.p, out2.ld, *s2);
+    MSK_LAUNCH_CHECK(ctx);
+    return 0;
+  }
   msk_launch_scope ls(ctx, "affine_act_fwd");
   if (sel.form != EwForm::CS && out2.p) {
     return msk_fail(ctx, __FILE__, __LINE__, "msk_affine_act_fwd_amax2", "the second output needs the channel-stationary float4 kernel (C / 4 a power of two, aligned tensors)");
@@ -1329,9 +1370,9 @@
                          (unsigned*)out_amax);
     });
   } else if (sel.form == EwForm::CS) {
-    hipLaunchKernelGGL(affine_act_fwd_cs_k, dim3(msk_ew_blocks(voxels * (x.c / 4) / 2, ctx->num_cu, g_ew_cap)), dim3(kThreads), 0, ctx->stream,
+    hipLaunchKernelGGL(affine_act_fwd_cs_k<false>, dim3(msk_ew_blocks(voxels * (x.c / 4) / 2, ctx->num_cu, g_ew_cap)), dim3(kThreads), 0, ctx->stream,
                        (const float*)x.p, x.ld, scale, shift, (const float*)res.p, res.ld, res.c, alpha, (float*)out.p,
-                       out.ld, voxels, x.c, sel.cshift, alpha_in, (unsigned*)out_amax, (float*)out2.p, out2.ld);
+                       out.ld, voxels, x.c, sel.cshift, alpha_in, (unsigned*)out_amax, (float*)out2.p, out2.ld, EwOut2Scale{});
   } else if (sel.form == EwForm::K4) {
     hipLaunchKernelGGL(affine_act_fwd_k<4>, dim3(msk_ew_blocks(voxels * x.c / 4, ctx->num_cu, g_ew_cap)), dim3(kThreads), 0,
                        ctx->stream, (const float*)x.p, x.ld, scale, shift, (const float*)res.p, res.ld, res.c,
@@ -1356,6 +1397,30 @@
                              const float* alpha, msk_tensor out, float* out_amax, msk_tensor out2) {
   if (out2.p) MSK_REQUIRE(ctx, msk_same_shape(x, out2) && vec4_ok(out2), "out2 must have x's shape and float4 alignment");
   return affine_act_fwd_impl(ctx, x, scale, shift, res, alpha, out, nullptr, out_amax, out2);
+}
+
+static int out2s_args(msk_ctx* ctx, msk_tensor x, msk_tensor out2, const float* out2_scale, float* out2_amax, EwOut2Scale* s2) {
+  MSK_REQUIRE(ctx, out2.p && msk_same_shape(x, out2), "out2 must have x's shape");
+  if (!vec4_ok(out2)) return 1;
+  s2->scale = out2_scale;
+  s2->vox_per_n = (long)x.d * x.h * x.w;
+  s2->amax = (unsigned*)out2_amax;
+  return 0;
+}
+int msk_affine_act_fwd_amax2s(msk_ctx* ctx, msk_tensor x, const float* scale, const float* shift, msk_tensor res, const float* alpha,
+                              msk_tensor out, float* out_amax, msk_tensor out2, const float* out2_scale, float* out2_amax) {
+  EwOut2Scale s2{};
+  if (int rc = out2s_args(ctx, x, out2, out2_scale, out2_amax, &s2)) return rc;
+  return affine_act_fwd_impl(ctx, x, scale, shift, res, alpha, out, nullptr, out_amax, out2, &s2);
+}
+int msk_affine_act_join_fwd_amax2s(msk_ctx* ctx, msk_tensor y, const float* scale, const float* shift, const float* alpha_inner,
+                                   msk_tensor res, const float* alpha_outer, msk_tensor out, float* out_amax, msk_tensor out2,
+                                   const float* out2_scale, float* out2_amax) {
+  MSK_REQUIRE(ctx, scale && shift && alpha_inner && alpha_outer && res.p, "join of a conv -> BN -> PReLU unit with a residual");
+  MSK_REQUIRE(ctx, res.c == y.c, "the residual has the unit's channel count");
+  EwOut2Scale s2{};
+  if (int rc = out2s_args(ctx, y, out2, out2_scale, out2_amax, &s2)) return rc;
+  return affine_act_fwd_impl(ctx, y, scale, shift, res, alpha_outer, out, alpha_inner, out_amax, out2, &s2);
 }
 
 int msk_affine_act_join_fwd_amax(msk_ctx* ctx, msk_tensor y, const float* scale, const float* shift, const float* alpha_inner,
@@ -1589,6 +1654,23 @@
   return 0;
 }
 
+int msk_dropout_masks(msk_ctx* ctx, uint64_t seed, uint64_t step, const msk_dropout_site* sites, int n) {
+  MSK_REQUIRE(ctx, sites != nullptr && n >= 1 && n <= MSK_DROPOUT_MAX_SITES, "msk_dropout_masks: 1 .. MSK_DROPOUT_MAX_SITES sites");
+  DropoutSites s{};
+  int most = 0;
+  for (int i = 0; i < n; ++i) {
+    MSK_REQUIRE(ctx, sites[i].p >= 0.f && sites[i].p < 1.f, "dropout p must be in [0,1)");
+    MSK_REQUIRE(ctx, sites[i].count >= 0 && (sites[i].mask != nullptr || sites[i].count == 0), "msk_dropout_masks: null mask");
+    s.e[i] = sites[i];
+    if (sites[i].count > most) most = sites[i].count;
+  }
+  if (most == 0) return 0;
+  msk_launch_scope ls(ctx, "dropout_masks");
+  hipLaunchKernelGGL(dropout_masks_k, dim3(msk_cdiv(most, 256), n), dim3(256), 0, ctx->stream, seed, step, s);
+  MSK_LAUNCH_CHECK(ctx);
+  return 0;
+}
+
 int msk_channel_sum(msk_ctx* ctx, msk_tensor x, float* out, int accumulate) {
   const long voxels = msk_voxels(x);
   const ReducePlan p = reduce_plan(PassTensors{x}, voxels, ctx->num_cu, 3, false);
diff --git a/medicalseg_amd/models/vnet.py b/medicalseg_amd/models/vnet.py
--- a/medicalseg_amd/models/vnet.py
+++ b/medicalseg_amd/models/vnet.py
@@ -87,19 +87,25 @@
         self._down = ConvBNAct(self.down_conv, self.bn1, self.relu1)
         self._join = AddAct(self.relu2)
 
-    def forward(self, x, out=None):
-        down = self._down.forward(x)
-        self._mask = self.dropout.make_mask(down) if self.if_dropout else None
+    def dropout_sites(self, n):
+        return [(self.dropout, n, self.down_conv.cout)] if self.if_dropout else []
+
+    def forward(self, x, out=None, drop=None):
+        self._mask = self.dropout.make_mask_nc(x.dev, x.n, self.down_conv.cout) if self.if_dropout else None
         if self._mask is not None:
-            t = down.empty_like()
-            copy_scale(down, self._mask, t)
+            od, oh, ow = self.down_conv.out_dims(x)
+            dropped = nn.DroppedOutput(Tensor.empty(x.dev, x.n, od, oh, ow, self.down_conv.cout), self._mask)
+            down = self._down.forward(x, drop=dropped)
+            t = dropped.t
+            if not dropped.filled:
+                copy_scale(down, self._mask, t)
         else:
-            t = down
+            t = down = self._down.forward(x)
         self._dropped = t
         self._t_down = down
         t, unit = _run_ops(self.ops, t, down)
         self._t_ops = t
-        return self._join.forward(t, down, unit=unit, out=out)
+        return self._join.forward(t, down, unit=unit, out=out, drop=drop)
 
     def backward(self, dout):
         down = self._t_down
@@ -132,6 +138,10 @@
         self._up = ConvBNAct(self.up_conv, self.bn1, self.relu1)
         self._join = AddAct(self.relu2)
 
+    def dropout_sites(self, n):
+        return ([(self.dropout1, n, self.up_conv.cin)] if self.if_dropout else []) + \
+               ([(self.dropout2, n, self.outChans - self.outChans // 2)] if self.if_dropout2 else [])
+
     def reserve_concat(self, dev, n, dims):
         self._reserved = None
         if self.if_dropout2 or os.environ.get("MSEGK_ZERO_COPY_SKIP", "1") == "0":
@@ -144,15 +154,51 @@
         self._reserved_skip = xcat.channel_slice(half, self.outChans)
         return self._reserved_skip
 
-    def forward(self, x, skipx):
+    def reserve_dropped_skip(self, dev, n, dims):
+        self._rs = None
+        mask = self.dropout2.make_mask_nc(dev, n, self.outChans - self.outChans // 2) if self.if_dropout2 else None
+        if mask is None:
+            return None
+        xcat = Tensor.empty(dev, n, dims[0], dims[1], dims[2], self.outChans)
+        if nn.PRODUCER_AMAX:
+            xcat.amax = dev.amax_new()
+        self._rs = nn.DroppedOutput(xcat.channel_slice(self.outChans // 2, self.outChans), mask)
+        self._rs.xcat = xcat
+        return self._rs
+
+    def reserve_dropped_x(self, dev, n, dims):
+        self._rx = None
+        mask = self.dropout1.make_mask_nc(dev, n, self.up_conv.cin) if self.if_dropout else None
+        if mask is None:
+            return None
+        self._rx = nn.DroppedOutput(Tensor.empty(dev, n, dims[0], dims[1], dims[2], self.up_conv.cin), mask)
+        return self._rx
+
+    def forward(self, x, skipx, drop=None):
         dev = x.dev
         self._x, self._skip = x, skipx
-        self._m1 = self.dropout1.make_mask(x) if self.if_dropout else None
-        self._m2 = self.dropout2.make_mask(skipx) if self.if_dropout2 else None
+        rx, rs = getattr(self, "_rx", None), getattr(self, "_rs", None)
+        self._rx = self._rs = None
+        if rx is not None and (rx.t.shape != x.shape or rx.t.gen != dev.arena.gen):
+            rx = nn.DroppedOutput(x.empty_like(), rx.mask)
+        if rs is not None and ((rs.t.n, rs.t.d, rs.t.h, rs.t.w, rs.t.c) != (skipx.n, skipx.d, skipx.h, skipx.w, skipx.c)
+                               or rs.t.gen != dev.arena.gen):
+            self._m2, rs = rs.mask, None
+        elif rs is not None:
+            self._m2 = rs.mask
+        else:
+            self._m2 = self.dropout2.make_mask(skipx) if self.if_dropout2 else None
+        if rx is not None:
+            self._m1 = rx.mask
+        else:
+            self._m1 = self.dropout1.make_mask(x) if self.if_dropout else None
         xin = x
         if self._m1 is not None:
-            xin = x.empty_like()
-            copy_scale(x, self._m1, xin)
+            if rx is None:
+                rx = nn.DroppedOutput(x.empty_like(), self._m1)
+            xin = rx.t
+            if not rx.filled:
+                copy_scale(x, self._m1, xin)
         self._xin = xin
         half = self.outChans // 2
         od, oh, ow = self.up_conv.out_dims(xin)
@@ -165,6 +211,8 @@
                                skipx.ptr == res.ptr + 4 * half and res.gen == dev.arena.gen)
         if self._skip_in_place:
             xcat, s_skip = res, skipx
+        elif rs is not None:
+            xcat, s_skip = rs.xcat, rs.t
         else:
             xcat = Tensor.empty(dev, x.n, od, oh, ow, self.outChans)
             if nn.PRODUCER_AMAX:
@@ -172,13 +220,13 @@
             s_skip = xcat.channel_slice(half, self.outChans)
         s_up = xcat.channel_slice(0, half)
         self._up.forward(xin, out=s_up)
-        if not self._skip_in_place:
+        if not self._skip_in_place and not (rs is not None and rs.filled):
             copy_scale(skipx, self._m2, s_skip)
         if xcat.amax is None or s_up.amax != xcat.amax or s_skip.amax != xcat.amax:
             xcat.amax = None
         self._xcat = xcat
         out, unit = _run_ops(self.ops, xcat, xcat)
-        return self._join.forward(out, xcat, unit=unit)
+        return self._join.forward(out, xcat, unit=unit, drop=drop)
 
     def join_for_consumer(self):
         ops = list(self.ops)
@@ -307,6 +355,12 @@
             else:
                 layer.injected, layer.enabled = None, False
 
+    def _draw_dropout_masks(self, n):
+        sites = []
+        for blk in (self.down_tr128, self.down_tr256, self.up_tr256, self.up_tr128):
+            sites += blk.dropout_sites(n)
+        nn.Dropout3D.draw_masks(self.dev, sites)
+
     def forward(self, x):
         if not isinstance(x, Tensor):
             x = to_tensor(x, self.dev)
@@ -315,7 +369,8 @@
         self.dev.arena.reset()
         if self.training:
             nn.Dropout3D.step += 1
-        slot = self.up_tr32.reserve_concat(self.dev, x.n, (x.d, x.h, x.w))
+            self._draw_dropout_masks(x.n)
+        slot =self.up_tr32.reserve_concat(self.dev, x.n, (x.d, x.h, x.w))
         twin = None
         if slot is not None and DENSE_TWIN and self.training and slot.c * 4 < 128 and not isinstance(self.in_tr.relu1, nn.ELU):
             twin = Tensor.empty(self.dev, x.n, x.d, x.h, x.w, slot.c)
@@ -323,10 +378,14 @@
         self._out16_twin = twin
         out32 = self.down_tr32(twin if twin is not None else out16,
                                out=self.up_tr64.reserve_concat(self.dev, x.n, self.down_tr32.down_conv.out_dims(out16)))
-        out64 = self.down_tr64(out32)
-        out128 = self.down_tr128(out64)
-        out256 = self.down_tr256(out128)
-        out = self.up_tr256(out256, out128)
+        dev, n = self.dev, x.n
+        d64 = self.down_tr64.down_conv.out_dims(out32)
+        out64 = self.down_tr64(out32, drop=self.up_tr128.reserve_dropped_skip(dev, n, d64))
+        d128 = self.down_tr128.down_conv.out_dims(out64)
+        out128 = self.down_tr128(out64, drop=self.up_tr256.reserve_dropped_skip(dev, n, d128))
+        d256 = self.down_tr256.down_conv.out_dims(out128)
+        out256 = self.down_tr256(out128, drop=self.up_tr256.reserve_dropped_x(dev, n, d256))
+        out = self.up_tr256(out256, out128, drop=self.up_tr128.reserve_dropped_x(dev, n, self.up_tr256.up_conv.out_dims(out256)))
         out = self.up_tr128(out, out64)
         out = self.up_tr64(out, out32)
         self._feat = self.up_tr32(out, out16)
diff --git a/medicalseg_amd/models/vnet_deepsup.py b/medicalseg_amd/models/vnet_deepsup.py
--- a/medicalseg_amd/models/vnet_deepsup.py
+++ b/medicalseg_amd/models/vnet_deepsup.py
@@ -77,6 +77,7 @@
         self.dev.arena.reset()
         if self.training:
             nn.Dropout3D.step += 1
+            self._draw_dropout_masks(x.n)
         size = (x.d, x.h, x.w)
         out16 = self.in_tr(x, out=self.up_tr32.reserve_concat(self.dev, x.n, (x.d, x.h, x.w)))
         out32 = self.down_tr32(out16, out=self.up_tr64.reserve_concat(self.dev, x.n, self.down_tr32.down_conv.out_dims(out16)))
diff --git a/medicalseg_amd/nn.py b/medicalseg_amd/nn.py
--- a/medicalseg_amd/nn.py
+++ b/medicalseg_amd/nn.py
@@ -392,17 +392,43 @@
         self.site = Dropout3D._site_counter
         self.injected = None
         self.enabled = True
+        self._drawn = None
+
+    def active(self):
+        return bool(self.training and self.enabled and self.p != 0.0)
+
+    @staticmethod
+    def draw_masks(dev, sites):
+        todo = []
+        batched = not getattr(dev.lib.msk_dropout_masks, "missing", False)
+        for layer, n, c in sites:
+            layer._drawn = None
+            if batched and layer.active() and layer.injected is None:
+                todo.append((layer, n, c))
+        for i in range(0, len(todo), _lib.DROPOUT_MAX_SITES):
+            part = todo[i:i + _lib.DROPOUT_MAX_SITES]
+            arr = (_lib.MskDropoutSite * len(part))()
+            for e, (layer, n, c) in zip(arr, part):
+                ptr = dev.arena.alloc(n * c * 4)
+                e.site, e.count, e.p, e.mask = layer.site | (dev.rank << 16), n * c, layer.p, ptr
+                layer._drawn = (ptr, n, c, dev.arena.gen)
+            dev.call("msk_dropout_masks", C.c_uint64(Dropout3D.seed), C.c_uint64(Dropout3D.step), C.cast(arr, C.c_void_p), len(part))
 
     def make_mask(self, x: Tensor):
-        if not self.training or not self.enabled or self.p == 0.0:
+        return self.make_mask_nc(x.dev, x.n, x.c)
+
+    def make_mask_nc(self, dev, n, c):
+        drawn, self._drawn = self._drawn, None
+        if not self.active():
             return None
-        dev = x.dev
-        cnt = x.n * x.c
+        if drawn is not None and self.injected is None and drawn[1:] == (n, c, dev.arena.gen):
+            return drawn[0]
+        cnt = n * c
         ptr = dev.arena.alloc(cnt * 4)
         if self.injected is not None:
             m = np.ascontiguousarray(self.injected, dtype=np.float32)
-            if m.shape != (x.n, x.c):
-                raise ValueError(f"injected dropout mask must be [{x.n},{x.c}], got {m.shape}")
+            if m.shape != (n, c):
+                raise ValueError(f"injected dropout mask must be [{n},{c}], got {m.shape}")
             dev.h2d(ptr, m)
         else:
             dev.call("msk_dropout_mask", C.c_uint64(Dropout3D.seed), C.c_uint64(Dropout3D.step),
@@ -452,6 +478,22 @@
 
 
 SHARE_JOIN_GRAD = os.environ.get("MSEGK_SHARE_JOIN_GRAD", "1") != "0"
+
+
+class DroppedOutput:
+
+    def __init__(self, t: Tensor, mask):
+        self.t, self.mask, self.filled = t, mask, False
+
+
+def _fused_drop(dev, name, *args) -> bool:
+    fn = getattr(dev.lib, name)
+    if getattr(fn, "missing", False):
+        return False
+    rc = fn(dev.ctx, *args)
+    if rc < 0:
+        raise MskError(f"{name} failed: {_lib.last_error(dev.ctx)}")
+    return rc == 0
 
 
 def materialize_grad(t: Tensor):
@@ -494,7 +536,8 @@
         self.x, self.res, self.y, self.out, self.bn_mode = x, None, None, out, 3
         return out
 
-    def forward(self, x: Tensor, res: Tensor | None = None, out: Tensor | None = None, defer_act=False, out2: Tensor | None = None) -> Tensor:
+    def forward(self, x: Tensor, res: Tensor | None = None, out: Tensor | None = None, defer_act=False, out2: Tensor | None = None,
+                drop: DroppedOutput | None = None) -> Tensor:
         dev = x.dev
         self.deferred = False
         if (_FUSED_INFERENCE["on"] and not self.bn.training and res is None and type(self.conv) is Conv3D
@@ -554,6 +597,11 @@
                          res.msk() if res is not None else NULL_TENSOR, _fp(alpha), out.msk())
                 dev.call("msk_elu_fwd", out.msk(), C.c_float(self.act.alpha), out.msk())
                 out.amax = None
+            elif (drop is not None and out2 is None and
+                  _fused_drop(dev, "msk_affine_act_fwd_amax2s", y.msk(), _fp(sc["scale"]), _fp(sc["shift"]),
+                              res.msk() if res is not None else NULL_TENSOR, _fp(alpha), out.msk(), _amax_for(out), drop.t.msk(),
+                              _fp(drop.mask), _amax_for(drop.t))):
+                drop.filled = True
             elif out2 is not None:
                 dev.call("msk_affine_act_fwd_amax2", y.msk(), _fp(sc["scale"]), _fp(sc["shift"]),
                          res.msk() if res is not None else NULL_TENSOR, _fp(alpha), out.msk(), _amax_for(out), out2.msk())
@@ -717,7 +765,8 @@
         self.act = act
         self._sums = None
 
-    def forward(self, a: Tensor, b: Tensor, unit: "ConvBNAct | None" = None, out: Tensor | None = None) -> Tensor:
+    def forward(self, a: Tensor, b: Tensor, unit: "ConvBNAct | None" = None, out: Tensor | None = None,
+                drop: DroppedOutput | None = None) -> Tensor:
         self.a, self.b = a, b
         self._bwd_done = False
         self.unit = unit if (unit is not None and getattr(unit, "deferred", False)) else None
@@ -731,8 +780,18 @@
             return out
         if self.unit is not None:
             u, sc = self.unit, self.unit.bn.scratch(a.dev)
-            a.dev.call("msk_affine_act_join_fwd_amax", u.y.msk(), _fp(sc["scale"]), _fp(sc["shift"]), _fp(u.act._weight.ptr),
-                       b.msk(), _fp(self.act._weight.ptr), out.msk(), _amax_for(out))
+            if (drop is not None and
+                    _fused_drop(a.dev, "msk_affine_act_join_fwd_amax2s", u.y.msk(), _fp(sc["scale"]), _fp(sc["shift"]),
+                                _fp(u.act._weight.ptr), b.msk(), _fp(self.act._weight.ptr), out.msk(), _amax_for(out), drop.t.msk(),
+                                _fp(drop.mask), _amax_for(drop.t))):
+                drop.filled = True
+            else:
+                a.dev.call("msk_affine_act_join_fwd_amax", u.y.msk(), _fp(sc["scale"]), _fp(sc["shift"]), _fp(u.act._weight.ptr),
+                           b.msk(), _fp(self.act._weight.ptr), out.msk(), _amax_for(out))
+        elif (drop is not None and
+              _fused_drop(a.dev, "msk_affine_act_fwd_amax2s", a.msk(), None, None, b.msk(), _fp(self.act._weight.ptr), out.msk(),
+                          _amax_for(out), drop.t.msk(), _fp(drop.mask), _amax_for(drop.t))):
+            drop.filled = True
         else:
             a.dev.call("msk_affine_act_fwd_amax", a.msk(), None, None, b.msk(), _fp(self.act._weight.ptr), out.msk(),
                        _amax_for(out))
```

Result: no change. 246.9 million (median of 4 runs) (+0.1%).
